# facebookresearch/nonrigid_nerf

Hardware: AMD Instinct MI355X
Metric: rendered rays/sec (64+128 samples/ray) (higher is better)
Workload: dtype bf16

## Files before the change

include/nrnerf.h:

```cpp
#ifndef NRNERF_H
#define NRNERF_H

#include <stddef.h>
#include <stdint.h>

#ifdef __cplusplus
extern "C" {
#endif

#define NRNERF_ABI_VERSION 10
#define NRNERF_MAX_SAMPLES 1024

typedef enum nrnerf_status {
    NRNERF_OK = 0,
    NRNERF_ERR_INVALID = -1,
    NRNERF_ERR_UNSUPPORTED = -2,
    NRNERF_ERR_HIP = -3,
    NRNERF_ERR_WORKSPACE = -4,
    NRNERF_ERR_NOMEM = -5,
    NRNERF_ERR_INTERNAL = -6
} nrnerf_status;

typedef enum nrnerf_precision {
    NRNERF_PREC_F32 = 0,
// ... 30 lines not shown
    int32_t rigidity_depth;
    int32_t rigidity_hidden;
    const nrnerf_linear* network;
    const nrnerf_linear* rigidity_network;
} nrnerf_bender_desc;

typedef struct nrnerf_model_desc {
    uint32_t struct_size;
    int32_t precision;
    int32_t multires;
    int32_t multires_views;
    int32_t device;
    const nrnerf_bender_desc* bender;
    const nrnerf_mlp_desc* coarse;
    const nrnerf_mlp_desc* fine;
    int32_t exact_viewdirs;
    uint32_t flags;
} nrnerf_model_desc;

typedef enum nrnerf_model_flags {
    NRNERF_MODEL_FORCE_GENERIC = 1u << 0,
    NRNERF_MODEL_NO_X16_F16 = 1u << 1
} nrnerf_model_flags;

typedef struct nrnerf_model nrnerf_model;

typedef struct nrnerf_sample_outputs {
    float* visibility_weights;
    float* opacity_alpha;
    float* initial_input_pts;
    float* unmasked_offsets;
    float* masked_offsets;
    float* input_pts;
    float* rigidity_mask;
} nrnerf_sample_outputs;

typedef struct nrnerf_render_args {
    uint32_t struct_size;
    int32_t n_rays;
    int32_t n_samples;
    int32_t n_importance;
    const float* rays;
    int32_t ray_stride;
    const float* latents;
    int32_t latent_stride;
    int32_t has_rigidity_cutoff;   float rigidity_cutoff;
    int32_t has_test_time_scaling; float test_time_scaling;
    int32_t has_removal_threshold; float removal_threshold;
    int32_t detailed_output;
    float* rgb_map;
    float* disp_map;
    float* acc_map;
    float* raw;
    float* rgb0;
    float* disp0;
    float* acc0;
    float* z_std;
    float* z_vals;
    float* surface_pts;
    float* surface_rigidity;
    int32_t* median_index;
    nrnerf_sample_outputs coarse;
    nrnerf_sample_outputs fine;
    void* workspace;
    size_t workspace_bytes;
    int32_t lindisp;
    int32_t white_bkgd;
    const float* u_coarse;
    const float* noise_coarse;
    const float* u_fine;
    const float* noise_fine;
    uint32_t flags;
} nrnerf_render_args;

typedef enum nrnerf_render_flags {
    NRNERF_RENDER_FUSED_FINE_BENDER = 1u << 0,
    NRNERF_RENDER_UNFUSED_COMPOSITE = 1u << 1,
    NRNERF_RENDER_SPLIT_COARSE = 1u << 2,
    NRNERF_RENDER_NO_X16 = 1u << 3,
    NRNERF_RENDER_X16_FINE_ONLY = 1u << 4,
    NRNERF_RENDER_BENDER_32X32 = 1u << 5,
    NRNERF_RENDER_COARSE_EPILOGUE_ON = 1u << 6,
    NRNERF_RENDER_COARSE_EPILOGUE_OFF = 1u << 7,
    NRNERF_RENDER_FIXED_SHARES = 1u << 8
} nrnerf_render_flags;

#define NRNERF_NUM_KERNELS 6
typedef struct nrnerf_profile {
    double ms[NRNERF_NUM_KERNELS];
    int64_t launches[NRNERF_NUM_KERNELS];
    double flops[NRNERF_NUM_KERNELS];
    double mfma_flops[NRNERF_NUM_KERNELS];
    char kernel_name[NRNERF_NUM_KERNELS][64];
} nrnerf_profile;

int nrnerf_abi_version(void);
const char* nrnerf_strerror(int status);

int nrnerf_model_create(const nrnerf_model_desc* desc, nrnerf_model** out);
int nrnerf_model_update(nrnerf_model* model, const nrnerf_model_desc* desc, void* hip_stream);
int64_t nrnerf_model_flat_size(const nrnerf_model* model);
int nrnerf_model_update_device(nrnerf_model* model, const float* flat_params, int64_t n_floats, void* hip_stream);
#define NRNERF_ADAM_MAX_SEGMENTS 40
typedef struct nrnerf_adam_segment {
    float* param; const float* grad; float* exp_avg; float* exp_avg_sq;
    uint64_t n;
} nrnerf_adam_segment;
typedef struct nrnerf_adam_args {
    uint32_t struct_size;
    int32_t n_segments;
    nrnerf_adam_segment segments[NRNERF_ADAM_MAX_SEGMENTS];
    float lr, beta1, beta2, eps;
    const float* lr_device;
    float* step;
    const float* flat_params;
    int64_t n_floats;
    uint32_t* barrier;
} nrnerf_adam_args;
int nrnerf_adam_step(nrnerf_model* model, const nrnerf_adam_args* args, void* hip_stream);

typedef struct nrnerf_tn_job {
    const void* a; const void* b;
    int32_t lda, ldb, wo, wi;
    int32_t ldo, reserved;
    int64_t out_offset, bias_offset;
} nrnerf_tn_job;
typedef struct nrnerf_tn_args {
    uint32_t struct_size;
    int32_t n_jobs, is_bf16, reserved;
    int64_t n_rows, out_floats;
    const nrnerf_tn_job* jobs;
    float* out;
    void* workspace; size_t workspace_bytes;
} nrnerf_tn_args;
size_t nrnerf_tn_workspace_bytes(const nrnerf_tn_args* args);
int nrnerf_tn_products(const nrnerf_tn_args* args, void* hip_stream);

typedef struct nrnerf_encoding_args {
    uint32_t struct_size;
    int32_t n_freqs;
    int64_t n_rows;
    const float* src; int32_t src_stride;
    void* enc; int32_t enc_cols; int32_t enc_is_bf16;
    const float* codes; int32_t n_lat; int32_t rows_per_code;
    const float* d_enc0; const float* d_enc1; int32_t d_enc_stride;
    float* d_src; int32_t d_src_stride;
} nrnerf_encoding_args;
int nrnerf_encoding_forward(const nrnerf_encoding_args* args, void* hip_stream);
int nrnerf_encoding_backward(const nrnerf_encoding_args* args, void* hip_stream);
void nrnerf_model_destroy(nrnerf_model* model);
int nrnerf_model_precision(const nrnerf_model* model);
int nrnerf_model_is_generic(const nrnerf_model* model);

size_t nrnerf_workspace_bytes(const nrnerf_model* model, int32_t n_rays, int32_t n_samples,
                              int32_t n_importance);

int nrnerf_render(const nrnerf_model* model, const nrnerf_render_args* args, void* hip_stream);

typedef struct nrnerf_camera {
    float c2w[12];
    float focal_x, focal_y, center_x, center_y;
    int32_t height, width;
} nrnerf_camera;
int nrnerf_generate_rays(const nrnerf_camera* cam, float near_plane, float far_plane, float* rays_out,
                         int32_t ray_stride, void* hip_stream);

int nrnerf_sample_depths(const float* rays, int32_t ray_stride, const float* uniforms, int32_t n_rays, int32_t n_samples,
// ... 123 lines not shown
    void* encv;
    float* head_sums;
} nrnerf_wgrad_args;
#define NRNERF_WGRAD_STRIDE_VIEWS(depth, width) (NRNERF_WGRAD_STRIDE(depth, width) + ((width) / 2) * (width) + 2 * ((width) / 2) * 64 + (width) / 2)
#define NRNERF_WGRAD_SHORT_PARTIALS(n_partials, width) \
    ((((n_partials) * (2 * ((width) / 64) + 2) + (2 * ((width) / 64) + (width) / 32) / 2) / (2 * ((width) / 64) + (width) / 32)) < 1 ? 1 : \
     (((n_partials) * (2 * ((width) / 64) + 2) + (2 * ((width) / 64) + (width) / 32) / 2) / (2 * ((width) / 64) + (width) / 32)))
#define NRNERF_WGRAD_STRIDE(depth, width) (((depth) - 1) * (width) * (width) + 3 * (width) * 64 + ((depth) + 1) * (width))
int nrnerf_trunk_wgrad(const nrnerf_model* model, const nrnerf_wgrad_args* args, void* hip_stream);

typedef struct nrnerf_generic_trunk_args {
    uint32_t struct_size;
    int32_t which;
    int32_t n_rays, n_samples;
    const float* pts4;
    void* acts;
    float* raw4;
    float* raw; int32_t raw_ch;
    const float* d_raw4;
    void* d_pre;
    float* d_enc0;
    float* d_enc1;
    const float* dirs;
    float* d_encv;
    const float* latents;
    void* relu_bits;
} nrnerf_generic_trunk_args;
size_t nrnerf_generic_trunk_bits_bytes(const nrnerf_model* model, int32_t which, int32_t n_rays, int32_t n_samples);
int nrnerf_generic_trunk_forward(const nrnerf_model* model, const nrnerf_generic_trunk_args* args, void* hip_stream);
int nrnerf_generic_trunk_backward(const nrnerf_model* model, const nrnerf_generic_trunk_args* args, void* hip_stream);
int nrnerf_model_trains_generic(const nrnerf_model* model);
int nrnerf_model_trains_bender(const nrnerf_model* model);

typedef struct nrnerf_loss_args {
    uint32_t struct_size;
    int32_t n_rays, n_samples;
    const float* rgb_map;
    const float* rgb0;
    const float* target;
    const float* weights;
    const float* offsets;
    const float* rigidity;
    const float* alpha;
    const float* divergence;
    float offsets_weight, rigidity_weight, divergence_weight;
    const float* schedule;
    float* loss;
    const float* g_loss;
    float* g_rgb_map;
    float* g_rgb0;
    float* g_offsets;
    float* g_rigidity;
    float* g_divergence;
    int32_t offsets_stride;
    int32_t rigidity_stride;
    const float* g_mean;
} nrnerf_loss_args;
int nrnerf_loss_forward(const nrnerf_loss_args* args, void* hip_stream);
int nrnerf_loss_backward(const nrnerf_loss_args* args, void* hip_stream);

int nrnerf_code_gradients(const int64_t* index, const float* g, int32_t n_rays, int32_t latent_size, int32_t n_codes, float* out, void* hip_stream);

typedef struct nrnerf_composite_args {
    uint32_t struct_size;
    int32_t n_rays, n_samples, n_importance;
    const float* rays; int32_t ray_stride;
    const float* raw4;
    const float* z;
    int32_t lindisp, white_bkgd;
    const float* noise;
    const float* u;
    float* rgb; float* disp; float* acc;
    float* weights; float* alpha;
    float* z_std; float* z_merged;
    const float* g_rgb; const float* g_disp; const float* g_acc; const float* g_weights;
    float* d_raw4;
    float* z_new;
    uint8_t* rank_new;
} nrnerf_composite_args;
int nrnerf_composite_forward(const nrnerf_composite_args* args, void* hip_stream);
int nrnerf_composite_backward(const nrnerf_composite_args* args, void* hip_stream);

int nrnerf_profile_begin(nrnerf_model* model);
int nrnerf_profile_end(nrnerf_model* model, nrnerf_profile* out);

typedef enum nrnerf_visualize_flags {
    NRNERF_VIS_DISP = 1, NRNERF_VIS_DISP_JET = 2, NRNERF_VIS_DISP_PHONG = 4,
    NRNERF_VIS_CORRESPONDENCES = 8, NRNERF_VIS_RIGIDITY = 16, NRNERF_VIS_RIGIDITY_JET = 32
} nrnerf_visualize_flags;
typedef enum nrnerf_visualize_normalize {
    NRNERF_VIS_NORM_NONE = 0,
    NRNERF_VIS_NORM_GIVEN = 1,
    NRNERF_VIS_NORM_FRAME = 2,
    NRNERF_VIS_NORM_STACK = 3
} nrnerf_visualize_normalize;
typedef struct nrnerf_visualize_args {
    uint32_t struct_size;
    uint32_t flags;
    int32_t n_frames, height, width;
    int32_t normalize;
    const float* disp;
    float* disp_max;
    const float* surface_pts;
    double min_point[3], max_point[3];
    int32_t voxels;
    const float* rigidity;
    uint8_t* disp_out;
    uint8_t* disp_jet;
    uint8_t* disp_phong;
    uint8_t* correspondences;
    uint8_t* rigidity_out;
    uint8_t* rigidity_jet;
} nrnerf_visualize_args;
int nrnerf_visualize_frames(const nrnerf_visualize_args* args, void* hip_stream);

typedef struct nrnerf_metrics_args {
    uint32_t struct_size;
    int32_t n_frames, height, width;
    const float* gt;
    const float* rendered;
    const float* mask_ref;
    double* psnr;
    double* ssim;
    double* mse;
    double* ssim_map;
    uint8_t* mse_error_map;
    uint8_t* ssim_error_map;
    void* workspace;
    size_t workspace_bytes;
} nrnerf_metrics_args;
size_t nrnerf_visualize_workspace_bytes(int32_t n_frames, int32_t height, int32_t width);
int nrnerf_image_metrics(const nrnerf_metrics_args* args, void* hip_stream);

int nrnerf_stability_accumulate(const float* rgb, int64_t n_values, double* sum, double* sum_sq, void* hip_stream);
int nrnerf_stability_finish(const double* sum, const double* sum_sq, int32_t n_frames, int64_t n_pixels, uint8_t* out_rgb, void* hip_stream);

typedef struct nrnerf_query_args {
    uint32_t struct_size;
    int32_t which;
    int32_t n_rows;
    int32_t n_samples;
    const float* points;
    int32_t point_stride;
    int32_t latent_stride;
    const float* latents;
    const float* viewdirs;
    int32_t has_rigidity_cutoff;   float rigidity_cutoff;
    int32_t has_test_time_scaling; float test_time_scaling;
    int32_t has_removal_threshold; float removal_threshold;
    int32_t detailed_output;
    uint32_t flags;
    int32_t raw_ch;
    float* raw;
    nrnerf_sample_outputs details;
    void* workspace;
    size_t workspace_bytes;
} nrnerf_query_args;
size_t nrnerf_query_workspace_bytes(const nrnerf_model* model, int32_t which, int32_t n_rows, int32_t n_samples);
int nrnerf_query(const nrnerf_model* model, const nrnerf_query_args* args, void* hip_stream);

int nrnerf_grid_points(const float min_point[3], const float max_point[3], int32_t gx, int32_t gy, int32_t gz, int64_t first_row,
                       int32_t n_rows, float* pts4, void* hip_stream);
int nrnerf_field_from_raw(const float* raw, int32_t raw_ch, int64_t n, float* sigma, uint8_t* rgb8, void* hip_stream);

typedef struct nrnerf_isosurface_args {
    uint32_t struct_size;
// ... 246 lines not shown
```

nonrigid_nerf_amd/_lib.py:

```python
from __future__ import annotations

import ctypes as C
import os

_HERE = os.path.dirname(os.path.abspath(__file__))
LIB_PATH = os.environ.get("NRNERF_LIB") or os.path.join(_HERE, "lib", "libnrnerf_hip.so")

ABI_VERSION = 10
MAX_SAMPLES = 1024
OK, ERR_INVALID, ERR_UNSUPPORTED, ERR_HIP, ERR_WORKSPACE, ERR_NOMEM, ERR_INTERNAL = 0, -1, -2, -3, -4, -5, -6
PRECISIONS = {"f32": 0, "fp32": 0, "float32": 0, "bf16": 1, "bfloat16": 1, "f16": 2, "fp16": 2, "float16": 2}
_CANONICAL = {0: "f32", 1: "bf16", 2: "f16"}


def canonical_precision(p: str) -> str:
    try:
        return _CANONICAL[PRECISIONS[p]]
    except KeyError:
        raise ValueError(f"unknown precision {p!r} (one of {sorted(PRECISIONS)})") from None
NUM_KERNELS = 6
KERNEL_NAMES = ("net_coarse", "composite_sample_coarse", "net_fine", "composite_fine", "bend_fine", "bend_coarse")

_fp = C.POINTER(C.c_float)


class Linear(C.Structure):
    _fields_ = [("weight", _fp), ("bias", _fp), ("out_features", C.c_int32), ("in_features", C.c_int32)]


class MlpDesc(C.Structure):
    _fields_ = [("depth", C.c_int32), ("width", C.c_int32), ("skip", C.c_int32), ("output_ch", C.c_int32),
                ("use_viewdirs", C.c_int32), ("time_conditioned", C.c_int32),
                ("pts_linears", C.POINTER(Linear)),
                ("output_linear", Linear), ("alpha_linear", Linear), ("feature_linear", Linear),
                ("views_linear", Linear), ("rgb_linear", Linear)]


class BenderDesc(C.Structure):
    _fields_ = [("latent_size", C.c_int32), ("depth", C.c_int32), ("hidden", C.c_int32),
                ("rigidity_depth", C.c_int32), ("rigidity_hidden", C.c_int32),
                ("network", C.POINTER(Linear)), ("rigidity_network", C.POINTER(Linear))]


class ModelDesc(C.Structure):
    _fields_ = [("struct_size", C.c_uint32), ("precision", C.c_int32), ("multires", C.c_int32),
                ("multires_views", C.c_int32), ("device", C.c_int32),
                ("bender", C.POINTER(BenderDesc)), ("coarse", C.POINTER(MlpDesc)), ("fine", C.POINTER(MlpDesc)),
                ("exact_viewdirs", C.c_int32), ("flags", C.c_uint32)]


class SampleOutputs(C.Structure):
    _fields_ = [(n, C.c_void_p) for n in ("visibility_weights", "opacity_alpha", "initial_input_pts",
                                           "unmasked_offsets", "masked_offsets", "input_pts", "rigidity_mask")]


class RenderArgs(C.Structure):
    _fields_ = [("struct_size", C.c_uint32), ("n_rays", C.c_int32), ("n_samples", C.c_int32),
                ("n_importance", C.c_int32),
                ("rays", C.c_void_p), ("ray_stride", C.c_int32),
                ("latents", C.c_void_p), ("latent_stride", C.c_int32),
                ("has_rigidity_cutoff", C.c_int32), ("rigidity_cutoff", C.c_float),
                ("has_test_time_scaling", C.c_int32), ("test_time_scaling", C.c_float),
                ("has_removal_threshold", C.c_int32), ("removal_threshold", C.c_float),
                ("detailed_output", C.c_int32),
                ("rgb_map", C.c_void_p), ("disp_map", C.c_void_p), ("acc_map", C.c_void_p), ("raw", C.c_void_p),
                ("rgb0", C.c_void_p), ("disp0", C.c_void_p), ("acc0", C.c_void_p), ("z_std", C.c_void_p),
                ("z_vals", C.c_void_p),
                ("surface_pts", C.c_void_p), ("surface_rigidity", C.c_void_p), ("median_index", C.c_void_p),
                ("coarse", SampleOutputs), ("fine", SampleOutputs),
                ("workspace", C.c_void_p), ("workspace_bytes", C.c_size_t),
                ("lindisp", C.c_int32), ("white_bkgd", C.c_int32),
                ("u_coarse", C.c_void_p), ("noise_coarse", C.c_void_p), ("u_fine", C.c_void_p), ("noise_fine", C.c_void_p),
                ("flags", C.c_uint32)]


MODEL_FORCE_GENERIC, MODEL_NO_X16_F16 = 1 << 0, 1 << 1
MODEL_PY_TRAINING_HANDLE = 1 << 30
RENDER_FUSED_FINE_BENDER, RENDER_UNFUSED_COMPOSITE, RENDER_SPLIT_COARSE, RENDER_NO_X16, RENDER_X16_FINE_ONLY, RENDER_BENDER_32X32, \
    RENDER_COARSE_EPILOGUE_ON, RENDER_COARSE_EPILOGUE_OFF, RENDER_FIXED_SHARES = (1 << i for i in range(9))


def model_flags_from_env() -> int:
    f = 0
    if os.environ.get("NRNERF_FORCE_GENERIC") == "1":
        f |= MODEL_FORCE_GENERIC
    if os.environ.get("NRNERF_X16_F16", "1") == "0":
        f |= MODEL_NO_X16_F16
    return f


_RENDER_ENV = ("NRNERF_FUSED_FINE_BENDER", "NRNERF_UNFUSED_COMPOSITE", "NRNERF_SPLIT_COARSE", "NRNERF_X16_BENDER", "NRNERF_X16",
               "NRNERF_FUSED_COARSE_EPILOGUE", "NRNERF_FIXED_SHARES")
_render_flags_cache = (None, 0)


def render_flags_from_env() -> int:
    global _render_flags_cache
    key = tuple(os.environ.get(k) for k in _RENDER_ENV)
    if _render_flags_cache[0] == key:
        return _render_flags_cache[1]
    f = 0
    if key[0] == "1":
        f |= RENDER_FUSED_FINE_BENDER
    if key[1] == "1":
        f |= RENDER_UNFUSED_COMPOSITE
    if key[2] == "1":
        f |= RENDER_SPLIT_COARSE
    if key[3] == "0":
        f |= RENDER_BENDER_32X32
    x16 = key[4]
    if x16 is not None and x16.strip() != "":
        if x16.strip() not in ("0", "1", "2"):
            raise ValueError(f"NRNERF_X16={x16!r}: one of 0 (32x32x16 kernels), 1 (16x16x32 fine pass only), 2 (both passes, the default)")
        f |= {0: RENDER_NO_X16, 1: RENDER_X16_FINE_ONLY}.get(int(x16), 0)
    if key[5] is not None and key[5].strip() != "":
        if key[5].strip() not in ("0", "1"):
            raise ValueError(f"NRNERF_FUSED_COARSE_EPILOGUE={key[5]!r}: 0 (composite / sample_pdf / merge as their own launch) or 1 (inside the coarse trunk kernel)")
        f |= RENDER_COARSE_EPILOGUE_ON if key[5].strip() == "1" else RENDER_COARSE_EPILOGUE_OFF
    if key[6] == "1":
        f |= RENDER_FIXED_SHARES
    _render_flags_cache = (key, f)
    return f


class GenericTrunkArgs(C.Structure):
    _fields_ = [("struct_size", C.c_uint32), ("which", C.c_int32), ("n_rays", C.c_int32), ("n_samples", C.c_int32),
                ("pts4", C.c_void_p), ("acts", C.c_void_p), ("raw4", C.c_void_p), ("raw", C.c_void_p), ("raw_ch", C.c_int32),
                ("d_raw4", C.c_void_p), ("d_pre", C.c_void_p), ("d_enc0", C.c_void_p), ("d_enc1", C.c_void_p),
                ("dirs", C.c_void_p), ("d_encv", C.c_void_p), ("latents", C.c_void_p), ("relu_bits", C.c_void_p)]


class LossArgs(C.Structure):
    _fields_ = [("struct_size", C.c_uint32), ("n_rays", C.c_int32), ("n_samples", C.c_int32),
                ("rgb_map", C.c_void_p), ("rgb0", C.c_void_p), ("target", C.c_void_p),
                ("weights", C.c_void_p), ("offsets", C.c_void_p), ("rigidity", C.c_void_p), ("alpha", C.c_void_p), ("divergence", C.c_void_p),
                ("offsets_weight", C.c_float), ("rigidity_weight", C.c_float), ("divergence_weight", C.c_float), ("schedule", C.c_void_p),
                ("loss", C.c_void_p), ("g_loss", C.c_void_p),
                ("g_rgb_map", C.c_void_p), ("g_rgb0", C.c_void_p), ("g_offsets", C.c_void_p), ("g_rigidity", C.c_void_p), ("g_divergence", C.c_void_p),
                ("offsets_stride", C.c_int32), ("rigidity_stride", C.c_int32), ("g_mean", C.c_void_p)]


class Profile(C.Structure):
    _fields_ = [("ms", C.c_double * NUM_KERNELS), ("launches", C.c_int64 * NUM_KERNELS),
                ("flops", C.c_double * NUM_KERNELS), ("mfma_flops", C.c_double * NUM_KERNELS),
                ("kernel_name", (C.c_char * 64) * NUM_KERNELS)]


class PackedInfo(C.Structure):
    _fields_ = [("stream_bytes", C.c_uint64), ("n_units", C.c_uint32), ("n_bias_tiles", C.c_uint32),
                ("frag_bytes", C.c_uint32), ("slot_bytes", C.c_uint32), ("mfma_per_block", C.c_uint32)]


class Camera(C.Structure):
    _fields_ = [("c2w", C.c_float * 12), ("focal_x", C.c_float), ("focal_y", C.c_float), ("center_x", C.c_float),
                ("center_y", C.c_float), ("height", C.c_int32), ("width", C.c_int32)]


class TrunkArgs(C.Structure):
    _fields_ = [("struct_size", C.c_uint32), ("which", C.c_int32), ("n_rays", C.c_int32), ("n_samples", C.c_int32),
                ("pts4", C.c_void_p), ("acts", C.c_void_p), ("relu_mask", C.c_void_p),
                ("raw4", C.c_void_p), ("raw", C.c_void_p), ("raw_ch", C.c_int32),
                ("d_raw4", C.c_void_p), ("d_pre", C.c_void_p), ("d_pts4", C.c_void_p), ("ray_bias", C.c_void_p),
                ("dirs", C.c_void_p), ("hv", C.c_void_p), ("hv_mask", C.c_void_p), ("d_pre_v", C.c_void_p), ("d_dirs", C.c_void_p)]


class WgradArgs(C.Structure):
    _fields_ = [("struct_size", C.c_uint32), ("n_rays", C.c_int32), ("n_samples", C.c_int32),
                ("acts", C.c_void_p), ("d_pre", C.c_void_p), ("pts4", C.c_void_p), ("d_raw4", C.c_void_p),
                ("enc", C.c_void_p), ("g_head", C.c_void_p),
                ("n_partials", C.c_int32), ("partials", C.c_void_p),
                ("dirs", C.c_void_p), ("hv", C.c_void_p), ("d_pre_v", C.c_void_p), ("encv", C.c_void_p), ("head_sums", C.c_void_p)]


REDUCE_SHORT = 0x40000000


def wgrad_stride(depth: int, width: int) -> int:
    return (depth - 1) * width * width + 3 * width * 64 + (depth + 1) * width


def wgrad_stride_views(depth: int, width: int) -> int:
    return wgrad_stride(depth, width) + (width // 2) * width + 2 * (width // 2) * 64 + width // 2


def wgrad_short_partials(n_partials: int, width: int) -> int:
    trw = width // 64
    return min(n_partials, max(1, (n_partials * (2 * trw + 2) + (2 * trw + width // 32) // 2) // (2 * trw + width // 32)))


class BenderArgs(C.Structure):
    _fields_ = [("struct_size", C.c_uint32), ("n_rays", C.c_int32), ("n_samples", C.c_int32),
                ("rays", C.c_void_p), ("ray_stride", C.c_int32),
                ("latents", C.c_void_p), ("latent_stride", C.c_int32),
                ("z", C.c_void_p),
                ("has_rigidity_cutoff", C.c_int32), ("rigidity_cutoff", C.c_float),
                ("has_test_time_scaling", C.c_int32), ("test_time_scaling", C.c_float),
                ("bent4", C.c_void_p), ("off4", C.c_void_p), ("acts_offsets", C.c_void_p), ("acts_rigidity", C.c_void_p),
                ("g_bent4", C.c_void_p), ("g_unmasked_offsets", C.c_void_p), ("g_rigidity_mask", C.c_void_p),
                ("dz_offsets", C.c_void_p), ("dz_rigidity", C.c_void_p), ("dz_out4", C.c_void_p), ("d_latents", C.c_void_p),
                ("g_bent4_b", C.c_void_p)]


class BenderWgradArgs(C.Structure):
# ... 203 lines not shown
                ("flags", C.c_uint32), ("bent4", C.c_void_p),
                ("workspace", C.c_void_p), ("workspace_bytes", C.c_size_t)]


BEND_POINTS_WORKSPACE_BYTES = 512 * 64


ISO_BLOCK, ISO_SCAN_CHUNK, ISO_MAX_VERTICES = 256, 4096, 1 << 30


def isosurface_workspace_bytes(gx: int, gy: int, gz: int) -> int:
    n = gx * gy * gz
    if min(gx, gy, gz) < 2 or n > ISO_MAX_VERTICES:
        return 0
    nb = (n + ISO_BLOCK - 1) // ISO_BLOCK
    return sum((b + 255) // 256 * 256 for b in (4 * n, 4 * nb, 4 * nb, 8 * nb, 8 * nb, n))


EXPORTS = {
    "nrnerf_abi_version": (C.c_int, []),
    "nrnerf_strerror": (C.c_char_p, [C.c_int]),
    "nrnerf_model_create": (C.c_int, [C.POINTER(ModelDesc), C.POINTER(C.c_void_p)]),
    "nrnerf_model_update": (C.c_int, [C.c_void_p, C.c_void_p, C.c_void_p]),
    "nrnerf_model_flat_size": (C.c_int64, [C.c_void_p]),
    "nrnerf_model_update_device": (C.c_int, [C.c_void_p, C.c_void_p, C.c_int64, C.c_void_p]),
    "nrnerf_adam_step": (C.c_int, [C.c_void_p, C.POINTER(AdamArgs), C.c_void_p]),
    "nrnerf_tn_workspace_bytes": (C.c_size_t, [C.POINTER(TnArgs)]),
    "nrnerf_tn_products": (C.c_int, [C.POINTER(TnArgs), C.c_void_p]),
    "nrnerf_encoding_forward": (C.c_int, [C.POINTER(EncodingArgs), C.c_void_p]),
    "nrnerf_encoding_backward": (C.c_int, [C.POINTER(EncodingArgs), C.c_void_p]),
    "nrnerf_model_destroy": (None, [C.c_void_p]),
    "nrnerf_model_precision": (C.c_int, [C.c_void_p]),
    "nrnerf_model_is_generic": (C.c_int, [C.c_void_p]),
    "nrnerf_generic_trunk_forward": (C.c_int, [C.c_void_p, C.POINTER(GenericTrunkArgs), C.c_void_p]),
    "nrnerf_generic_trunk_backward": (C.c_int, [C.c_void_p, C.POINTER(GenericTrunkArgs), C.c_void_p]),
    "nrnerf_model_trains_generic": (C.c_int, [C.c_void_p]),
    "nrnerf_generic_trunk_bits_bytes": (C.c_size_t, [C.c_void_p, C.c_int32, C.c_int32, C.c_int32]),
    "nrnerf_model_trains_bender": (C.c_int, [C.c_void_p]),
    "nrnerf_loss_forward": (C.c_int, [C.POINTER(LossArgs), C.c_void_p]),
    "nrnerf_loss_backward": (C.c_int, [C.POINTER(LossArgs), C.c_void_p]),
    "nrnerf_code_gradients": (C.c_int, [C.c_void_p, C.c_void_p, C.c_int32, C.c_int32, C.c_int32, C.c_void_p, C.c_void_p]),
    "nrnerf_workspace_bytes": (C.c_size_t, [C.c_void_p, C.c_int32, C.c_int32, C.c_int32]),
    "nrnerf_render": (C.c_int, [C.c_void_p, C.POINTER(RenderArgs), C.c_void_p]),
    "nrnerf_query_workspace_bytes": (C.c_size_t, [C.c_void_p, C.c_int32, C.c_int32, C.c_int32]),
    "nrnerf_query": (C.c_int, [C.c_void_p, C.POINTER(QueryArgs), C.c_void_p]),
    "nrnerf_grid_points": (C.c_int, [_fp, _fp, C.c_int32, C.c_int32, C.c_int32, C.c_int64, C.c_int32, C.c_void_p, C.c_void_p]),
    "nrnerf_field_from_raw": (C.c_int, [C.c_void_p, C.c_int32, C.c_int64, C.c_void_p, C.c_void_p, C.c_void_p]),
    "nrnerf_isosurface_workspace_bytes": (C.c_size_t, [C.c_int32, C.c_int32, C.c_int32]),
    "nrnerf_isosurface_count": (C.c_int, [C.POINTER(IsosurfaceArgs), C.c_void_p]),
    "nrnerf_isosurface_emit": (C.c_int, [C.POINTER(IsosurfaceArgs), C.c_void_p]),
    "nrnerf_bender_inverse_workspace_bytes": (C.c_size_t, [C.c_void_p]),
    "nrnerf_bender_inverse": (C.c_int, [C.c_void_p, C.POINTER(BenderInverseArgs), C.c_void_p]),
    "nrnerf_volume_render": (C.c_int, [C.POINTER(VolumeRenderArgs), C.c_void_p]),
    "nrnerf_warped_volume_render": (C.c_int, [C.POINTER(WarpedVolumeRenderArgs), C.c_void_p]),
    "nrnerf_grid_lookup_backward": (C.c_int, [C.POINTER(GridLookupBackwardArgs), C.c_void_p]),
    "nrnerf_sh_volume_render": (C.c_int, [C.POINTER(ShVolumeRenderArgs), C.c_void_p]),
    "nrnerf_occupancy_words": (C.c_int64, [C.POINTER(C.c_int32), C.c_int32]),
    "nrnerf_occupancy_build": (C.c_int, [C.POINTER(OccupancyBuildArgs), C.c_void_p]),
    "nrnerf_culled_volume_render": (C.c_int, [C.POINTER(CulledVolumeRenderArgs), C.c_void_p]),
    "nrnerf_bend_points_workspace_bytes": (C.c_size_t, [C.c_void_p]),
    "nrnerf_bend_points": (C.c_int, [C.c_void_p, C.POINTER(BendPointsArgs), C.c_void_p]),
    "nrnerf_generate_rays": (C.c_int, [C.POINTER(Camera), C.c_float, C.c_float, C.c_void_p, C.c_int32, C.c_void_p]),
    "nrnerf_sample_depths": (C.c_int, [C.c_void_p, C.c_int32, C.c_void_p, C.c_int32, C.c_int32, C.c_int32, C.c_void_p, C.c_void_p]),
    "nrnerf_sample_depths_points": (C.c_int, [C.c_void_p, C.c_int32, C.c_void_p, C.c_int32, C.c_int32, C.c_int32, C.c_void_p, C.c_void_p, C.c_void_p]),
    "nrnerf_merge_rows": (C.c_int, [C.c_void_p, C.c_int32, C.c_int32, C.c_int32, C.c_void_p, C.c_void_p, C.c_void_p, C.c_void_p, C.c_void_p, C.c_void_p,
                                    C.c_int32, C.c_void_p]),
    "nrnerf_reduce_partials": (C.c_int, [C.c_void_p, C.c_int64, C.c_int32, C.c_int32, C.c_void_p, C.c_int64, C.c_void_p, C.c_void_p]),
    "nrnerf_reduce_partials_aux": (C.c_int, [C.c_void_p, C.c_int64, C.c_int32, C.c_int32, C.c_void_p, C.c_int64, C.c_void_p, C.c_void_p, C.c_int32,
                                             C.POINTER(C.c_int64), C.c_void_p]),
    "nrnerf_tile_row_sums": (C.c_int, [C.c_void_p, C.c_int64, C.c_void_p, C.c_void_p]),
    "nrnerf_tiles_to_rows": (C.c_int, [C.c_void_p, C.c_int32, C.c_int32, C.c_int32, C.c_void_p, C.c_void_p]),
    "nrnerf_direction_encoding": (C.c_int, [C.c_void_p, C.c_int32, C.c_int32, C.c_int32, C.c_void_p, C.c_int32, C.c_void_p, C.c_void_p]),
    "nrnerf_trunk_forward": (C.c_int, [C.c_void_p, C.POINTER(TrunkArgs), C.c_void_p]),
    "nrnerf_trunk_backward": (C.c_int, [C.c_void_p, C.POINTER(TrunkArgs), C.c_void_p]),
    "nrnerf_trunk_wgrad": (C.c_int, [C.c_void_p, C.POINTER(WgradArgs), C.c_void_p]),
    "nrnerf_bender_forward": (C.c_int, [C.c_void_p, C.POINTER(BenderArgs), C.c_void_p]),
    "nrnerf_bender_backward": (C.c_int, [C.c_void_p, C.POINTER(BenderArgs), C.c_void_p]),
    "nrnerf_bender_wgrad": (C.c_int, [C.c_void_p, C.POINTER(BenderWgradArgs), C.c_void_p]),
    "nrnerf_bender_divergence_forward": (C.c_int, [C.c_void_p, C.POINTER(DivergenceArgs), C.c_void_p]),
    "nrnerf_bender_divergence_backward": (C.c_int, [C.c_void_p, C.POINTER(DivergenceArgs), C.c_void_p]),
    "nrnerf_composite_forward": (C.c_int, [C.POINTER(CompositeArgs), C.c_void_p]),
    "nrnerf_composite_backward": (C.c_int, [C.POINTER(CompositeArgs), C.c_void_p]),
    "nrnerf_profile_begin": (C.c_int, [C.c_void_p]),
    "nrnerf_profile_end": (C.c_int, [C.c_void_p, C.POINTER(Profile)]),
    "nrnerf_visualize_frames": (C.c_int, [C.POINTER(VisualizeArgs), C.c_void_p]),
    "nrnerf_visualize_workspace_bytes": (C.c_size_t, [C.c_int32, C.c_int32, C.c_int32]),
    "nrnerf_image_metrics": (C.c_int, [C.POINTER(MetricsArgs), C.c_void_p]),
    "nrnerf_stability_accumulate": (C.c_int, [C.c_void_p, C.c_int64, C.c_void_p, C.c_void_p, C.c_void_p]),
    "nrnerf_stability_finish": (C.c_int, [C.c_void_p, C.c_void_p, C.c_int32, C.c_int64, C.c_void_p, C.c_void_p]),
    "nrnerf_pack_host": (C.c_int, [C.POINTER(ModelDesc), C.c_int, C.POINTER(PackedInfo), C.c_void_p, C.c_size_t,
                                   C.POINTER(C.c_uint32), _fp]),
}

_lib = None


class NrnerfError(RuntimeError):
    def __init__(self, status: int, where: str):
        self.status = status
        super().__init__(f"{where}: {strerror(status)} (status {status})")


def load() -> C.CDLL:
    global _lib
    if _lib is None:
        if not os.path.exists(LIB_PATH):
            raise ImportError(
                f"{LIB_PATH} not found: build it with `python -c 'import __graft_entry__ as g; g.build()'` "
                "(or `make -C nonrigid_nerf_amd/csrc -j8`). nonrigid_nerf_amd has no CPU fallback.")
        import torch
        lib = C.CDLL(LIB_PATH)
        for name, (res, args) in EXPORTS.items():
            fn = getattr(lib, name)
            fn.restype, fn.argtypes = res, args
        v = lib.nrnerf_abi_version()
        if v != ABI_VERSION:
            raise ImportError(f"libnrnerf_hip.so ABI version {v}, binding expects {ABI_VERSION}")
        _lib = lib
    return _lib


def strerror(status: int) -> str:
    return load().nrnerf_strerror(status).decode()


def check(status: int, where: str):
    if status != OK:
        raise NrnerfError(status, where)
```

nonrigid_nerf_amd/csrc/nrnerf_api.cpp:

```cpp
#include <hip/hip_runtime.h>

#include <cstdio>
#include <cstring>
#include <mutex>
#include <new>
#include <vector>

#include "nrnerf_model.h"
#include "nrnerf_aux.h"
#include "nrnerf_x16_api.h"
#include "nrnerf_plan.h"
#include "nrnerf_bend_points.h"
#include "nrnerf_field.h"

using namespace nrn;

namespace {

int upload_pass(const PackedPass& pk, PassDev& dev) {
    dev.stream_bytes = pk.stream.size();
    dev.bias_floats = pk.bias.size();
    if (hipMalloc(&dev.stream, pk.stream.size()) != hipSuccess) return NRNERF_ERR_NOMEM;
    if (hipMalloc((void**)&dev.bias, pk.bias.size() * 4) != hipSuccess) return NRNERF_ERR_NOMEM;
    if (hipMemcpy(dev.stream, pk.stream.data(), pk.stream.size(), hipMemcpyHostToDevice) != hipSuccess) return NRNERF_ERR_HIP;
// ... 344 lines not shown
    }
    template <class F> hipError_t timed(nrnerf_model::Ev ev, F&& launch) {
        if (!prof) return launch();
        if (hipEventCreateWithFlags(&ev.a, hipEventDisableSystemFence) != hipSuccess ||
            hipEventCreateWithFlags(&ev.b, hipEventDisableSystemFence) != hipSuccess) return hipErrorUnknown;
        (void)hipEventRecord(ev.a, stream);
        const hipError_t e = launch();
        (void)hipEventRecord(ev.b, stream);
        std::lock_guard<std::mutex> g(m->prof_mu);
        m->prof_events.push_back(ev);
        return e;
    }
    hipError_t run_program(const nrnerf_model::Ev& ev, const GenArgs& g) { return timed(ev, [&] { return launch_generic(m->precision, g, m->num_cus, stream); }); }
    static SampleOut sample_out(const nrnerf_sample_outputs& o) {
        return SampleOut{o.visibility_weights, o.opacity_alpha, o.initial_input_pts, o.unmasked_offsets, o.masked_offsets, o.input_pts, o.rigidity_mask};
    }
    const nrnerf_sample_outputs& outputs_of(const PassPlan& p) const { return p.which ? a->fine : a->coarse; }
    const float* depths_of(const PassPlan& p) const { return p.which ? z_fine : zc; }
    float* points_of(const PassPlan& p) const { return p.final ? bent4_ws : bent_c; }
    float* raw_of(const PassPlan& p) const { return p.which ? raw_f : raw_c; }

    hipError_t bender_step(const PassPlan& p) {
        const float* const zv = p.bend_rank ? z_new : depths_of(p);
        if (p.bend == BendStep::Program) {
            const ImageDev& im = m->gen_bend;
            GenArgs g = im.prog;
            g.rays = a->rays; g.ray_stride = a->ray_stride; g.latents = a->latents; g.lat_stride = a->latent_stride;
            g.z = zv; g.lindisp = a->lindisp; g.n_rays = N; g.S = p.bend_n;
            g.wstream = im.stream; g.bias = im.bias;
            g.bent4 = points_of(p); g.ex = sample_out(outputs_of(p)); g.knobs = kn;
            return run_program(work(p.bend_slot, "gen_kernel (bender program)", im, p.bend_n), g);
        }
        const ImageDev& im = plan.bend_x16 ? m->bend_x16 : m->bend_only;
        BendArgs b{};
        b.rays = a->rays; b.ray_stride = a->ray_stride; b.latents = a->latents; b.lat_stride = a->latent_stride;
        b.z = zv; b.lindisp = a->lindisp; b.rank = p.bend_rank ? rank_new : nullptr; b.n_rays = N; b.n_per_ray = p.bend_n; b.out_stride = p.bend_stride;
        b.wstream = im.stream; b.bias = im.bias; b.bent4 = points_of(p); b.knobs = kn;
        b.work_counter = counter(p.bend_dynamic, (size_t)16 * BEND_COUNTERS_PER_LAUNCH * p.which);
        return timed(work(p.bend_slot, plan.bend_x16 ? "bend_kernel_x16" : "bend_kernel", im, p.bend_n), [&] {
            return plan.bend_x16 ? launch_bend_x16(bender_arch_of(m), b, m->num_cus, stream) : launch_bend(m->precision, bender_arch_of(m), b, m->num_cus, stream);
        });
    }
    CompositeArgs composite_args(const PassPlan& p) const {
        const bool fine = p.which == 1;
        const nrnerf_sample_outputs& so = outputs_of(p);
        CompositeArgs c{};
        c.rays = a->rays; c.ray_stride = a->ray_stride;
        c.raw4 = raw_of(p); c.z = depths_of(p); c.n_rays = N; c.S = p.S; c.n_importance = p.final ? 0 : I;
        c.lindisp = a->lindisp; c.white_bkgd = a->white_bkgd; c.noise = fine ? a->noise_fine : a->noise_coarse;
        c.vis = so.visibility_weights; c.alpha = so.opacity_alpha;
        if (p.final) {
            c.rgb = a->rgb_map; c.disp = a->disp_map; c.acc = a->acc_map; c.z_user = a->z_vals;
            if (plan.surface) { c.bent4 = bent4_ws; c.surf_pts = a->surface_pts; c.surf_rig = a->surface_rigidity; c.med_idx = a->median_index; }
        } else {
            c.u = a->u_fine;
            c.rgb = a->rgb0 ? a->rgb0 : raw_f; c.disp = a->disp0 ? a->disp0 : raw_f + (size_t)N * 3; c.acc = a->acc0 ? a->acc0 : raw_f + (size_t)N * 4;
            c.z_std = a->z_std; c.z_out = z_fine;
            if (plan.split) { c.split_bent_in = bent_c; c.split_bent_out = bent4_ws; c.z_new = z_new; c.rank_new = rank_new; }
        }
        return c;
    }
    hipError_t network_step(const PassPlan& p, const CompositeArgs& c) {
        const bool fused = p.comp != CompStep::Launch;
        const ImageDev& im = m->img[p.image];
        const nrnerf_sample_outputs& so = outputs_of(p);
        const float* const pts = given_pts ? given_pts : ((p.bend == BendStep::Compiled || p.bend == BendStep::Program) ? points_of(p) : nullptr);
        float* const pts_out = (!pts && (p.final ? plan.surface : plan.split)) ? points_of(p) : nullptr;
        float* const raw4 = fused ? nullptr : raw_of(p);
        float* const raw_out = p.final ? a->raw : nullptr;
        CompositeArgs fuse = fused ? c : CompositeArgs{};
        fuse.raw4 = nullptr;
        const nrnerf_model::Ev ev = work(p.net_slot, p.name, im, p.S);
        switch (p.net) {
        case NetFamily::NetBender: case NetFamily::NetTrunk: case NetFamily::NetX16: {
            NetArgs n{};
            n.rays = a->rays; n.ray_stride = a->ray_stride; n.latents = a->latents; n.lat_stride = a->latent_stride;
            n.z = depths_of(p); n.lindisp = a->lindisp; n.pts4 = pts; n.n_rays = N; n.S = p.S;
            n.wstream = im.stream; n.bias = im.bias;
            n.raw4 = raw4; n.raw_out = raw_out; n.raw_ch = im.output_ch; n.bent4 = pts_out;
            n.ex = sample_out(so); n.knobs = kn; n.fuse_on = fused; n.fuse = fuse;
            return timed(ev, [&] {
                if (p.net != NetFamily::NetX16) return launch_net(m->precision, p.net == NetFamily::NetBender, m->views, p.dispatch, n, m->num_cus, stream);
                n.work_counter = counter(p.trunk_counter, (size_t)16 * BEND_COUNTERS_PER_LAUNCH * 2 + 16 * p.which);
                return launch_net_x16(m->precision, p.dispatch, m->views, n, m->num_cus, stream);
            });
        }
        case NetFamily::Gx16: {
            const GxMeta& gm = im.gx;
            GxArgs x{};
            x.pts4 = pts; x.raw4 = raw4; x.raw_out = raw_out; x.raw_ch = im.output_ch;
            x.n_rays = N; x.S = p.S; x.wstream = im.stream; x.bias = im.bias;
            x.depth = gm.depth; x.skip = gm.skip; x.L = gm.L; x.n_bias_tiles = gm.n_bias_tiles; x.LV = gm.LV;
            x.fuse_on = fused; x.fuse = fuse;
            return timed(ev, [&] { return launch_gx16(m->precision, p.dispatch, gm.views != 0, x, m->num_cus, stream); });
        }
        case NetFamily::Gen: {
            GenArgs g = im.prog;
            g.rays = a->rays; g.ray_stride = a->ray_stride; g.latents = a->latents; g.lat_stride = a->latent_stride;
            g.z = depths_of(p); g.lindisp = a->lindisp; g.n_rays = N; g.S = p.S;
            g.pts4 = pts; g.dirs_from_pts = (pts && m->views && m->has_bend) ? 1 : 0;
            g.wstream = im.stream; g.bias = im.bias;
            g.raw4 = raw4; g.raw_out = raw_out; g.raw_ch = im.output_ch;
            g.bent4 = pts ? const_cast<float*>(pts) : pts_out;
            g.knobs = kn;
            if (!pts) g.ex = sample_out(so);
            return run_program(ev, g);
        }
        case NetFamily::GenExact: {
            BendDivArgs t{};
            t.latents = a->latents; t.lat_stride = a->latent_stride; t.m = (long long)N * p.S;
            t.wstream = m->bend_train_fwd.stream; t.bias = m->bend_train_fwd.bias;
            t.knobs.has_cutoff = kn.has_cutoff; t.knobs.cutoff = kn.cutoff; t.knobs.has_scaling = kn.has_scaling; t.knobs.scaling = kn.scaling;
            t.rays = a->rays; t.ray_stride = a->ray_stride; t.zr = depths_of(p); t.S = p.S; t.lindisp = a->lindisp; t.dirs_out = jdirs;
            const bool b16 = m->precision != NRNERF_PREC_F32;
            const hipError_t je = (m->gen_compiled_bender == 0) ? launch_bend_div_fwd_a0(t, m->num_cus, stream, b16) : launch_bend_div_fwd_a1(t, m->num_cus, stream, b16);
            if (je != hipSuccess) return je;
            GenArgs g = im.prog;
            g.mode = 1;
            g.rays = pts; g.ray_stride = 0; g.latents = nullptr; g.lat_stride = 0;
            g.z = nullptr; g.lindisp = 0; g.n_rays = N; g.S = p.S;
            g.pts4 = pts; g.dirs_from_pts = 0; g.dirs = jdirs;
            g.wstream = im.stream; g.bias = im.bias;
            g.raw4 = raw4; g.raw_out = raw_out; g.raw_ch = im.output_ch; g.bent4 = const_cast<float*>(pts);
            g.save = nullptr; g.mask = nullptr; g.save_stride = 0; g.save_w = 0;
            g.knobs = kn;
            return timed(ev, [&] { return launch_generic_train(m->precision, g, m->num_cus, stream); });
        }
        }
        return hipErrorUnknown;
    }
    int run_pass(const PassPlan& p) {
        if ((p.bend == BendStep::Compiled || p.bend == BendStep::Program) && bender_step(p) != hipSuccess) return NRNERF_ERR_HIP;
        const CompositeArgs c = composite_args(p);
        if (network_step(p, c) != hipSuccess) return NRNERF_ERR_HIP;
        if (p.comp != CompStep::Launch) return NRNERF_OK;
        const nrnerf_model::Ev ev{p.net_slot + 1, nullptr, nullptr, 0, 0, "composite_kernel"};
        return status_of(timed(ev, [&] { return launch_composite(c, stream); }));
    }
};
}
extern "C" {

int nrnerf_render(const nrnerf_model* m, const nrnerf_render_args* a, void* hip_stream) try {
    if (!m || !a || a->struct_size != sizeof(nrnerf_render_args)) return NRNERF_ERR_INVALID;
    if (a->n_rays < 0 || a->n_samples < 2 || a->n_importance < 0) return NRNERF_ERR_INVALID;
    if (a->n_samples > NRNERF_MAX_SAMPLES || a->n_samples + a->n_importance > NRNERF_MAX_SAMPLES) return NRNERF_ERR_UNSUPPORTED;
    if (a->n_rays == 0) return NRNERF_OK;
    if (!a->rays || a->ray_stride < 8 || !a->rgb_map || !a->disp_map || !a->acc_map) return NRNERF_ERR_INVALID;
    if (m->needs_latents && (!a->latents || a->latent_stride < 0)) return NRNERF_ERR_INVALID;
    if (m->views && (!m->has_bend || m->exact) && a->ray_stride < 11) return NRNERF_ERR_INVALID;
    const size_t need = nrnerf_workspace_bytes(m, a->n_rays, a->n_samples, a->n_importance);
    if (!a->workspace || a->workspace_bytes < need || ((uintptr_t)a->workspace & 255)) return NRNERF_ERR_WORKSPACE;
    hipStream_t stream = (hipStream_t)hip_stream;
    DeviceGuard guard(m->device);
    if (!guard.ok) return NRNERF_ERR_HIP;
    const WorkspaceLayout lay(a->n_rays, a->n_samples, a->n_importance, m->generic && m->exact);
    if ((a->u_fine || a->noise_fine) && a->n_importance == 0) return NRNERF_ERR_INVALID;
    const RenderPlan plan = plan_render(*m, *a);
    RenderCall call(m, a, plan, lay, stream);
    if (plan.counters_first) (void)call.counter(true, 0);
    if (a->u_coarse) {
        JitterArgs ja{a->rays, a->ray_stride, a->u_coarse, a->n_rays, a->n_samples, a->lindisp, call.z_coarse};
        if (launch_zjitter(ja, stream) != hipSuccess) return NRNERF_ERR_HIP;
        call.zc = call.z_coarse;
    }
    const int rc = call.run_pass(plan.coarse);
// ... 129 lines not shown
        r.n_rays = (int32_t)M; r.n_samples = 1; r.rays = pk.point_records;
        if (q.point_latents) { r.latents = pk.latents_out; r.latent_stride = m->latent_size; }
    }
    RenderPlan rp;
    rp.generic = m->generic != 0; rp.bend_x16 = q.bend_x16;
    RenderCall call(m, &r, rp, stream, raw4, pts4, (unsigned*)(ws + lay.counters));
    if (p.bend_dynamic) (void)call.counter(true, 0);
    if (!q.per_point && !m->has_bend) call.given_pts = pts4;

    if (p.bend == BendStep::Compiled) {
        const ImageDev& bi = q.bend_x16 ? m->bend_x16 : m->bend_only;
        BendPointArgs b{};
        b.b.latents = a->latents; b.b.lat_stride = a->latent_stride; b.b.n_rays = N; b.b.n_per_ray = S; b.b.out_stride = S;
        b.b.wstream = bi.stream; b.b.bias = bi.bias; b.b.bent4 = pts4; b.b.knobs = call.kn;
        b.b.work_counter = call.counter(p.bend_dynamic, (size_t)16 * BEND_COUNTERS_PER_LAUNCH * p.which);
        b.src.points = a->points; b.src.stride = a->point_stride; b.src.unmasked = d.unmasked_offsets; b.src.masked = d.masked_offsets;
        const hipError_t e = call.timed(call.work(p.bend_slot, q.bend_x16 ? "bend_kernel_x16 (point source)" : "bend_kernel (point source)", bi, S), [&] {
            return q.bend_x16 ? launch_bend_points_x16(bender_arch_of(m), b, m->num_cus, stream)
                              : launch_bend_points(m->precision, bender_arch_of(m), b, m->num_cus, stream);
        });
        if (e != hipSuccess) return NRNERF_ERR_HIP;
    }
    if (call.network_step(p, CompositeArgs{}) != hipSuccess) return NRNERF_ERR_HIP;
    if (m->has_bend) {
        QueryUnpackArgs u{};
        u.bent4 = pts4; u.n = M; u.in_pts = d.input_pts; u.rigidity = d.rigidity_mask;
        u.raw = a->raw; u.raw_ch = a->raw_ch; u.has_removal = a->detailed_output && a->has_removal_threshold; u.removal = a->removal_threshold;
        if ((u.in_pts || u.rigidity || u.has_removal) && launch_query_unpack(u, stream) != hipSuccess) return NRNERF_ERR_HIP;
    }
    return NRNERF_OK;
} NRN_CATCH

int nrnerf_grid_points(const float min_point[3], const float max_point[3], int32_t gx, int32_t gy, int32_t gz, int64_t first_row,
                       int32_t n_rows, float* pts4, void* hip_stream) try {
    if (!min_point || !max_point || gx < 1 || gy < 1 || gz < 1 || first_row < 0 || n_rows < 0) return NRNERF_ERR_INVALID;
    if (first_row + n_rows > (int64_t)gy * gz) return NRNERF_ERR_INVALID;
    if (n_rows == 0) return NRNERF_OK;
    if (!pts4) return NRNERF_ERR_INVALID;
    GridArgs g{};
    for (int c = 0; c < 3; ++c) { g.lo[c] = min_point[c]; g.hi[c] = max_point[c]; }
    g.g[0] = gx; g.g[1] = gy; g.g[2] = gz; g.first_row = first_row; g.n_rows = n_rows; g.pts4 = pts4;
    return on_owner_of(pts4, [&] { return status_of(launch_grid_points(g, (hipStream_t)hip_stream)); });
} NRN_CATCH

int nrnerf_field_from_raw(const float* raw, int32_t raw_ch, int64_t n, float* sigma, uint8_t* rgb8, void* hip_stream) try {
    if (n < 0 || raw_ch < 4) return NRNERF_ERR_INVALID;
    if (n == 0 || (!sigma && !rgb8)) return NRNERF_OK;
    if (!raw) return NRNERF_ERR_INVALID;
    return on_owner_of(raw, [&] { return status_of(launch_field_from_raw(raw, raw_ch, n, sigma, rgb8, (hipStream_t)hip_stream)); });
} NRN_CATCH

int nrnerf_generate_rays(const nrnerf_camera* cam, float near_plane, float far_plane, float* rays_out,
                         int32_t ray_stride, void* hip_stream) try {
    if (!cam || !rays_out || (ray_stride != 8 && ray_stride != 11)) return NRNERF_ERR_INVALID;
    if (cam->height <= 0 || cam->width <= 0 || cam->focal_x == 0.0f || cam->focal_y == 0.0f) return NRNERF_ERR_INVALID;
    RayGenArgs a{};
    std::memcpy(a.c2w, cam->c2w, sizeof(a.c2w));
    a.fx = cam->focal_x; a.fy = cam->focal_y; a.cx = cam->center_x; a.cy = cam->center_y;
    a.H = cam->height; a.W = cam->width; a.near = near_plane; a.far = far_plane;
    a.rays = rays_out; a.ray_stride = ray_stride;
    return on_owner_of(rays_out, [&] { return status_of(launch_raygen(a, (hipStream_t)hip_stream)); });
} NRN_CATCH

int nrnerf_sample_depths(const float* rays, int32_t ray_stride, const float* uniforms, int32_t n_rays, int32_t n_samples,
                         int32_t lindisp, float* z_out, void* hip_stream) try {
    if (!rays || !z_out || ray_stride < 8 || n_rays < 0 || n_samples < 2 || n_samples > NRNERF_MAX_SAMPLES) return NRNERF_ERR_INVALID;
    if (n_rays == 0) return NRNERF_OK;
    const JitterArgs j{rays, ray_stride, uniforms, n_rays, n_samples, lindisp, z_out};
    return on_owner_of(z_out, [&] { return status_of(launch_zjitter(j, (hipStream_t)hip_stream)); });
} NRN_CATCH
int nrnerf_sample_depths_points(const float* rays, int32_t ray_stride, const float* uniforms, int32_t n_rays, int32_t n_samples,
                                int32_t lindisp, float* z_out, float* points_out, void* hip_stream) try {
    if (!rays || !z_out || !points_out || ray_stride < 8 || n_rays < 0 || n_samples < 2 || n_samples > NRNERF_MAX_SAMPLES) return NRNERF_ERR_INVALID;
    if (n_rays == 0) return NRNERF_OK;
    const SamplePointsArgs j{rays, ray_stride, uniforms, n_rays, n_samples, lindisp, z_out, points_out};
    return on_owner_of(z_out, [&] { return status_of(launch_sample_points(j, (hipStream_t)hip_stream)); });
} NRN_CATCH

int nrnerf_profile_begin(nrnerf_model* m) try {
    if (!m) return NRNERF_ERR_INVALID;
    std::lock_guard<std::mutex> g(m->prof_mu);
    for (auto& e : m->prof_events) { (void)hipEventDestroy(e.a); (void)hipEventDestroy(e.b); }
    m->prof_events.clear();
    m->prof_on = true;
    return NRNERF_OK;
} NRN_CATCH

int nrnerf_profile_end(nrnerf_model* m, nrnerf_profile* out) try {
    if (!m || !out) return NRNERF_ERR_INVALID;
    std::lock_guard<std::mutex> g(m->prof_mu);
    m->prof_on = false;
    std::memset(out, 0, sizeof(*out));
    int rc = NRNERF_OK;
    for (auto& e : m->prof_events) {
        float ms = 0.f;
        if (hipEventSynchronize(e.b) != hipSuccess || hipEventElapsedTime(&ms, e.a, e.b) != hipSuccess) rc = NRNERF_ERR_HIP;
        out->ms[e.kernel] += ms;
        out->launches[e.kernel] += 1;
        out->flops[e.kernel] += e.flops;
        out->mfma_flops[e.kernel] += e.mfma;
        if (e.name) std::snprintf(out->kernel_name[e.kernel], sizeof(out->kernel_name[e.kernel]), "%s", e.name);
        (void)hipEventDestroy(e.a); (void)hipEventDestroy(e.b);
    }
    m->prof_events.clear();
    return rc;
} NRN_CATCH

}
```

nonrigid_nerf_amd/csrc/nrnerf_kernels.h:

```cpp
#pragma once
#include <hip/hip_runtime.h>
#include <stdint.h>

#include <type_traits>

namespace nrn {

constexpr int epl_class(int S) {
    const int n = (S + 63) / 64;
    return n <= 4 ? n : n <= 6 ? 6 : n <= 8 ? 8 : n <= 12 ? 12 : 16;
}
static_assert(epl_class(1) == 1 && epl_class(64) == 1 && epl_class(65) == 2 && epl_class(128) == 2 && epl_class(129) == 3 && epl_class(192) == 3 &&
              epl_class(193) == 4 && epl_class(256) == 4 && epl_class(257) == 6 && epl_class(384) == 6 && epl_class(385) == 8 && epl_class(512) == 8 &&
              epl_class(513) == 12 && epl_class(768) == 12 && epl_class(769) == 16 && epl_class(1024) == 16, "the lane-width table");
template <class F>
auto with_epl(int S, F&& f) {
    switch (epl_class(S)) {
        case 1: return f(std::integral_constant<int, 1>{});
        case 2: return f(std::integral_constant<int, 2>{});
        case 3: return f(std::integral_constant<int, 3>{});
        case 4: return f(std::integral_constant<int, 4>{});
        case 6: return f(std::integral_constant<int, 6>{});
        case 8: return f(std::integral_constant<int, 8>{});
        case 12: return f(std::integral_constant<int, 12>{});
        default: return f(std::integral_constant<int, 16>{});
    }
}

struct SampleOut {
    float* vis;
    float* alpha;
    float* init_pts;
    float* unmasked;
    float* masked;
    float* in_pts;
    float* rigidity;
};

struct Knobs {
    int has_cutoff;  float cutoff;
    int has_scaling; float scaling;
    int has_removal; float removal;
    int detailed;
};

struct CompositeArgs {
    const float* rays;   int ray_stride;
    const float* raw4;
    const float* z;
    int lindisp;
    int white_bkgd;
    const float* noise;
    const float* u;
    int n_rays, S;
    int n_importance;
    float* rgb; float* disp; float* acc;
    float* z_std;
    float* z_out;
    float* z_user;
    float* vis; float* alpha;
    const float* bent4;
    float* surf_pts;
    float* surf_rig;
    int* med_idx;
    const float* split_bent_in;
    float* split_bent_out;
    float* z_new;
    uint8_t* rank_new;
};

struct NetArgs {
    const float* rays;   int ray_stride;
    const float* latents; int lat_stride;
    const float* z;
    int lindisp;
    const float* pts4;
    int n_rays, S;
    const void* wstream;
    const float* bias;
    float* raw4;
    float* raw_out;
    int raw_ch;
    float* bent4;
    SampleOut ex;
    Knobs knobs;
    int fuse_on;
    CompositeArgs fuse;
    unsigned* work_counter;
};



struct BendArgs {
    const float* rays;   int ray_stride;
    const float* latents; int lat_stride;
    const float* z;
    int lindisp;
    const uint8_t* rank;
    int n_rays, n_per_ray, out_stride;
    const void* wstream;
    const float* bias;
    float* bent4;
    Knobs knobs;
    unsigned* work_counter;
};
hipError_t launch_bend(int precision, int arch_id, const BendArgs& a, int num_cus, hipStream_t stream);

struct CompositeBwdArgs {
    const float* rays;   int ray_stride;
    const float* raw4;
    const float* z;
    int lindisp, white_bkgd;
    const float* noise;
    int n_rays, S;
    const float* g_rgb;
    const float* g_disp;
    const float* g_acc;
    const float* g_w;
    float* d_raw4;
};
hipError_t launch_composite_bwd(const CompositeBwdArgs& a, hipStream_t stream);

struct TrunkArgs {
    const float* pts4;
    int n_rays, S;
    const void* wstream;
    const float* bias;
    float* raw4;
    float* raw_out;
    int raw_ch;
    void* acts;
    unsigned short* mask;
    const float* d_raw4;
    const float* ray_bias;
    void* d_pre;
    float* d_pts4;
    const float* dirs;
    void* hv;
    unsigned short* hv_mask;
    void* d_pre_v;
    float* d_dirs;
};

hipError_t launch_trunk_fwd_train_f32(const TrunkArgs&, int num_cus, hipStream_t);
hipError_t launch_trunk_fwd_train_bf16(const TrunkArgs&, int num_cus, hipStream_t);
hipError_t launch_trunk_bwd_f32(const TrunkArgs&, int num_cus, hipStream_t);
hipError_t launch_trunk_bwd_bf16(const TrunkArgs&, int num_cus, hipStream_t);
hipError_t launch_trunk_fwd_train_f32_views(const TrunkArgs&, int num_cus, hipStream_t);
hipError_t launch_trunk_fwd_train_bf16_views(const TrunkArgs&, int num_cus, hipStream_t);
hipError_t launch_trunk_bwd_f32_views(const TrunkArgs&, int num_cus, hipStream_t);
hipError_t launch_trunk_bwd_bf16_views(const TrunkArgs&, int num_cus, hipStream_t);
hipError_t launch_trunk_fwd_train_f32_a5(const TrunkArgs&, int num_cus, hipStream_t);
hipError_t launch_trunk_fwd_train_bf16_a5(const TrunkArgs&, int num_cus, hipStream_t);
hipError_t launch_trunk_bwd_f32_a5(const TrunkArgs&, int num_cus, hipStream_t);
hipError_t launch_trunk_bwd_bf16_a5(const TrunkArgs&, int num_cus, hipStream_t);

struct BendTrainArgs {
    const float* rays;   int ray_stride;
    const float* latents; int lat_stride;
    const float* z;
    int n_rays, S;
    const void* wstream;
    const float* bias;
    Knobs knobs;
    float* bent4;
    float* off4;
    void* acts_b;
    void* acts_r;
    const float* g_bent4;
    const float* g_bent4_b;
    const float* g_unmasked;
// ... 192 lines not shown
```

nonrigid_nerf_amd/csrc/nrnerf_model.h:

```cpp
#pragma once
#include <hip/hip_runtime.h>

#include <mutex>
#include <new>
#include <vector>

#include "nrnerf_pack.h"

#define NRN_CATCH catch (const std::bad_alloc&) { return NRNERF_ERR_NOMEM; } catch (...) { return NRNERF_ERR_INTERNAL; }

struct PassDev {
    void* stream = nullptr;
    float* bias = nullptr;
    size_t stream_bytes = 0, bias_floats = 0;
    double algo_flops_per_sample = 0;
    double mfma_flops_per_sample = 0;
    int output_ch = 4;
    int32_t* src = nullptr; int32_t* bias_src = nullptr; uint8_t* fmt = nullptr;
    size_t n_elems = 0;
};

struct ImageDev : PassDev { nrn::GenArgs prog{}; nrn::GxMeta gx{}; };

struct DeviceGuard {
    int prev = -1;
    bool ok = true;
    explicit DeviceGuard(int want) {
        if (hipGetDevice(&prev) != hipSuccess) { ok = false; prev = -1; return; }
        if (prev != want && hipSetDevice(want) != hipSuccess) ok = false;
        if (prev == want) prev = -1;
    }
    ~DeviceGuard() { if (prev >= 0) (void)hipSetDevice(prev); }
};

struct nrnerf_model : nrn::ModelTraits {
    explicit nrnerf_model(const nrn::ModelTraits& t)
        : nrn::ModelTraits(t), fine(img[t.fine_is_coarse ? nrn::IMG_COARSE : nrn::IMG_FINE]), gen_fine(img[t.fine_is_coarse ? nrn::IMG_GEN_COARSE : nrn::IMG_GEN_FINE]) {}
    int device = 0, num_cus = 0;
    ImageDev img[nrn::IMG_COUNT];
    ImageDev &coarse = img[nrn::IMG_COARSE], &fine;
    ImageDev &fine_trunk = img[nrn::IMG_FINE_TRUNK], &coarse_trunk = img[nrn::IMG_COARSE_TRUNK], &bend_only = img[nrn::IMG_BEND_ONLY];
    ImageDev &fine_trunk_x16 = img[nrn::IMG_FINE_TRUNK_X16], &coarse_trunk_x16 = img[nrn::IMG_COARSE_TRUNK_X16];
    ImageDev &bend_x16 = img[nrn::IMG_BEND_X16];
    ImageDev &coarse_bwd = img[nrn::IMG_COARSE_BWD], &fine_bwd = img[nrn::IMG_FINE_BWD];
    ImageDev &coarse_train = img[nrn::IMG_COARSE_TRAIN], &fine_train = img[nrn::IMG_FINE_TRAIN];
    ImageDev &bend_train_fwd = img[nrn::IMG_BEND_TRAIN_FWD], &bend_train_bwd = img[nrn::IMG_BEND_TRAIN_BWD];
    ImageDev &gen_bend = img[nrn::IMG_GEN_BEND], &gen_coarse = img[nrn::IMG_GEN_COARSE], &gen_fine;
    ImageDev &gx_coarse = img[nrn::IMG_GX_COARSE], &gx_fine = img[nrn::IMG_GX_FINE];
    ImageDev &gen_coarse_bwd = img[nrn::IMG_GEN_COARSE_BWD], &gen_fine_bwd = img[nrn::IMG_GEN_FINE_BWD];
    ImageDev &gx_coarse_bwd = img[nrn::IMG_GX_COARSE_BWD], &gx_fine_bwd = img[nrn::IMG_GX_FINE_BWD];
    int64_t flat_floats = 0;
    unsigned* adam_barrier = nullptr;
    mutable std::mutex prof_mu;
    mutable bool prof_on = false;
    struct Ev { int kernel; hipEvent_t a, b; double flops, mfma; const char* name; };
    mutable std::vector<Ev> prof_events;
};

namespace nrn { hipError_t launch_generic_train(int precision, const GenArgs& a, int num_cus, hipStream_t stream); }

inline int bender_arch_of(const nrnerf_model* m) { return m->generic ? m->gen_compiled_bender : nrn::bender_arch(m->arch_id); }

inline int device_of(const void* ptr, int& dev) {
    hipPointerAttribute_t attr;
    if (hipPointerGetAttributes(&attr, ptr) != hipSuccess) { (void)hipGetLastError(); return NRNERF_ERR_INVALID; }
    if (attr.type != hipMemoryTypeDevice) return NRNERF_ERR_INVALID;
    dev = attr.device;
    return NRNERF_OK;
}

inline int status_of(hipError_t e) { return e == hipSuccess ? NRNERF_OK : NRNERF_ERR_HIP; }
inline int status_of_checked_launch(hipError_t e) { return e == hipErrorInvalidValue ? NRNERF_ERR_INVALID : status_of(e); }

template <class RUN> int on_device(int dev, RUN&& run) {
    DeviceGuard guard(dev);
    if (!guard.ok) return NRNERF_ERR_HIP;
    return run();
}
template <class RUN> int on_owner_of(const void* ptr, RUN&& run) {
    int dev = 0;
    if (device_of(ptr, dev) != NRNERF_OK) return NRNERF_ERR_INVALID;
    return on_device(dev, run);
}
template <class RUN> int on_model_device(const nrnerf_model* m, RUN&& run) { return on_device(m->device, run); }

inline int repack_batches(const nrnerf_model* m, const float* flat_params, hipStream_t stream) {
    for (const ImageDev& p : m->img)
        if (p.stream && !p.src) return NRNERF_ERR_UNSUPPORTED;
    nrn::RepackBatchArgs b{};
    b.flat = flat_params;
    auto add = [&](const int32_t* src, const uint8_t* fmt, void* dst, long long n) -> bool {
        if (n <= 0) return true;
        if (b.n_segments == nrn::REPACK_MAX_SEGMENTS) {
            if (nrn::launch_repack_batch(b, stream) != hipSuccess) return false;
            b.n_segments = 0;
        }
        const int k = b.n_segments++;
        if (k == 0) b.block0[0] = 0;
        b.src[k] = src; b.fmt[k] = fmt; b.dst[k] = dst; b.n[k] = n;
        b.block0[k + 1] = b.block0[k] + (unsigned)((n + 255) / 256);
        return true;
    };
    for (const ImageDev& p : m->img) {
        if (!p.stream) continue;
        if (!add(p.src, p.fmt, p.stream, (long long)p.n_elems) || !add(p.bias_src, nullptr, p.bias, (long long)p.bias_floats)) return NRNERF_ERR_HIP;
    }
    return status_of(nrn::launch_repack_batch(b, stream));
}
```

nonrigid_nerf_amd/csrc/nrnerf_net_impl.h:

```cpp
#pragma once
#include <hip/hip_runtime.h>
#include <type_traits>

#include "nrnerf_kernels.h"
#include "nrnerf_plan.h"
#include "nrnerf_composite_ray.h"

#ifndef NRN_PF16
#define NRN_PF16 4
#endif
#ifndef NRN_EPI_DELAY
#define NRN_EPI_DELAY 4
#endif

namespace nrn {

#ifdef NRN_TIMING
static __device__ unsigned long long g_nrn_timing[8][8];
#define NRN_NOW() __builtin_amdgcn_s_memtime()
#define NRN_TACC(slot, t0) tacc[slot] += NRN_NOW() - (t0)
#else
#define NRN_NOW() 0ull
#define NRN_TACC(slot, t0) ((void)0)
#endif
// ... 2 lines not shown
typedef float f32x4 __attribute__((ext_vector_type(4)));

template <int I, int N, class F>
__device__ __forceinline__ void static_for(F&& f) {
    if constexpr (N - I == 1) {
        f(std::integral_constant<int, I>{});
    } else if constexpr (N - I > 1) {
        constexpr int M = I + (N - I) / 2;
        static_for<I, M>(f);
        static_for<M, N>(f);
    }
}

typedef short s16x8 __attribute__((ext_vector_type(8)));
typedef short s16x2 __attribute__((ext_vector_type(2)));
typedef float f32x2 __attribute__((ext_vector_type(2)));
typedef unsigned u32x4 __attribute__((ext_vector_type(4)));

template <class F8, class F2, int U, bool RELU>
__device__ __forceinline__ F8 pack16(const f32x16& c) {
    u32x4 w;
#pragma unroll
    for (int k = 0; k < 4; ++k) {
        const f32x2 t = {c[8 * U + 2 * k], c[8 * U + 2 * k + 1]};
        const F2 p = __builtin_convertvector(t, F2);
        s16x2 q = __builtin_bit_cast(s16x2, p);
        if (RELU) q = __builtin_elementwise_max(q, (s16x2)(short)0);
        w[k] = __builtin_bit_cast(unsigned, q);
    }
    return __builtin_bit_cast(F8, w);
}

__device__ __forceinline__ float relu_bits(float x) {
    return __builtin_bit_cast(float, max(__builtin_bit_cast(int, x), 0));
}
struct PolBF16 : Shape<8, false> {
    typedef __bf16 frag __attribute__((ext_vector_type(8)));
    static constexpr int PF = NRN_PF16;
    typedef __bf16 frag2 __attribute__((ext_vector_type(2)));
    template <int U, bool RELU>
    static __device__ __forceinline__ frag from_acc(const f32x16& c) { return pack16<frag, frag2, U, RELU>(c); }
    static __device__ __forceinline__ f32x16 mfma(frag a, frag b, f32x16 c) {
        return __builtin_amdgcn_mfma_f32_32x32x16_bf16(a, b, c, 0, 0, 0);
    }
    template <int E>
    static __device__ __forceinline__ void set(frag& f, float v) { f[E] = (__bf16)v; }
    static __device__ __forceinline__ float round(float v) { return (float)(__bf16)v; }
};
struct PolF16 : Shape<8, true> {
    typedef _Float16 frag __attribute__((ext_vector_type(8)));
    static constexpr int PF = NRN_PF16;
    typedef _Float16 frag2 __attribute__((ext_vector_type(2)));
    template <int U, bool RELU>
    static __device__ __forceinline__ frag from_acc(const f32x16& c) { return pack16<frag, frag2, U, RELU>(c); }
    static __device__ __forceinline__ f32x16 mfma(frag a, frag b, f32x16 c) {
        return __builtin_amdgcn_mfma_f32_32x32x16_f16(a, b, c, 0, 0, 0);
    }
    template <int E>
    static __device__ __forceinline__ void set(frag& f, float v) { f[E] = (_Float16)v; }
    static __device__ __forceinline__ float round(float v) { return (float)(_Float16)v; }
};
struct PolF32 : Shape<1> {
    typedef float frag;
    static constexpr int PF = 8;
    template <int U, bool RELU>
    static __device__ __forceinline__ frag from_acc(const f32x16& c) { return RELU ? relu_bits(c[U]) : c[U]; }
    static __device__ __forceinline__ f32x16 mfma(frag a, frag b, f32x16 c) {
        return __builtin_amdgcn_mfma_f32_32x32x2f32(a, b, c, 0, 0, 0);
    }
    template <int E>
    static __device__ __forceinline__ void set(frag& f, float v) { f = v; }
    static __device__ __forceinline__ float round(float v) { return v; }
};

#ifndef NRN_RING_LAG
#define NRN_RING_LAG 2
#endif
template <int N>
__device__ __forceinline__ void wait_ring() {
    if constexpr (NRN_RING_LAG == 1) asm volatile("s_waitcnt vmcnt(%0) lgkmcnt(0)" ::"n"(N) : "memory");
    else asm volatile("s_waitcnt vmcnt(%0)" ::"n"(N) : "memory");
}

template <class P, int WAVES, int NUP>
struct WRing {
    static constexpr int UNIT = P::UNIT_BYTES;
    static constexpr int PW = UNIT / 1024 / WAVES;
    static constexpr int LAG = NRN_RING_LAG;
    static_assert(LAG >= 1 && RING - LAG >= 2, "need at least one unit of DMA lead");
    static_assert(UNIT % (1024 * WAVES) == 0, "unit must split evenly over the waves");
    static_assert(NUP % RING == 0 && NUP >= RING, "unit count must be a padded multiple of the ring depth");
    const char* ubase;
    unsigned lane16;
    char* ring;
    int wave_off;
    int lane_off;
    unsigned lane_addr;
#ifdef NRN_TIMING
    unsigned long long bar_cycles = 0, bar_count = 0;
#endif

    __device__ __forceinline__ void init(const void* stream, char* lds, int wave, int lane) {
        wave_off = wave * PW * 1024;
        ubase = (const char*)stream + wave_off;
        lane16 = (unsigned)lane * 16u;
        ring = lds;
        lane_off = lane * (P::FRAG_BYTES / 64);
        lane_addr = (unsigned)(size_t)(__attribute__((address_space(3))) char*)lds + (unsigned)lane_off;
        static_for<0, RING - LAG>([&](auto uc) { issue<decltype(uc)::value>(); });
    }
    template <int V>
    __device__ __forceinline__ void issue() {
        unsigned off = (unsigned)(V * UNIT);
        asm volatile("" : "+s"(off));
        const char* src = (ubase + off) + lane16;
        char* dst = ring + (V % RING) * UNIT + wave_off;
        static_for<0, PW>([&](auto ic) {
            __builtin_amdgcn_global_load_lds((const __attribute__((address_space(1))) void*)src,
                                             (__attribute__((address_space(3))) void*)dst, 16, decltype(ic)::value * 1024, 0);
        });
    }
    template <int U>
    __device__ __forceinline__ void advance() {
#ifdef NRN_TIMING
        const unsigned long long tb0 = NRN_NOW();
#endif
        wait_ring<(RING - LAG - 1) * PW>();
        __builtin_amdgcn_s_barrier();
        asm volatile("" ::: "memory");
#ifdef NRN_TIMING
        bar_cycles += NRN_NOW() - tb0; ++bar_count;
#endif
        issue<(U + RING - LAG) % NUP>();
    }
    static constexpr bool ASM_FRAGS = (P::FRAG_BYTES == 1024);
    template <class PX, int GF>
    __device__ __forceinline__ typename PX::frag frag() {
        static_assert(PX::FRAG_BYTES == P::FRAG_BYTES, "mixed policies must share the fragment size");
        constexpr int UF = P::UNIT_FRAGS;
        if constexpr (GF % UF == 0) advance<GF / UF>();
        constexpr int OFF = ((GF / UF) % RING) * UNIT + (GF % UF) * P::FRAG_BYTES;
        if constexpr (ASM_FRAGS) {
            static_assert(OFF + 16 <= 65536, "ring must stay within the immediate ds_read offset");
            u32x4 v;
            asm volatile("ds_read_b128 %0, %1 offset:%2" : "=v"(v) : "v"(lane_addr), "n"(OFF));
            return __builtin_bit_cast(typename PX::frag, v);
        } else {
            const char* p = ring + OFF + lane_off;
            return *(const typename PX::frag*)p;
        }
    }
    template <int N, class F>
    __device__ __forceinline__ void ready(F& f) {
        if constexpr (ASM_FRAGS) {
            static_assert(N >= 0 && N <= 15, "lgkmcnt is a 4-bit counter");
            u32x4 v = __builtin_bit_cast(u32x4, f);
            asm volatile("s_waitcnt lgkmcnt(%1)" : "+v"(v) : "n"(N));
            f = __builtin_bit_cast(F, v);
        }
    }
    __device__ __forceinline__ void drain() { asm volatile("s_waitcnt vmcnt(0)" ::: "memory"); }
};

typedef const __attribute__((address_space(3))) f32x4* BiasPtr;
__device__ __forceinline__ BiasPtr bias_lane_ptr(const float* bias_lds, int h) {
    BiasPtr p = (BiasPtr)(bias_lds + h * 16);
    asm volatile("" : "+v"(p));
    return p;
}
__device__ __forceinline__ f32x16 load_bias(BiasPtr bias_lane, int tile) {
    BiasPtr bp = bias_lane + tile * 8;
    const f32x4 b0 = bp[0], b1 = bp[1], b2 = bp[2], b3 = bp[3];
    return f32x16{b0[0], b0[1], b0[2], b0[3], b1[0], b1[1], b1[2], b1[3],
                  b2[0], b2[1], b2[2], b2[3], b3[0], b3[1], b3[2], b3[3]};
}

template <int NT, int NS>
struct SeqPos {
    static constexpr int NPAIR = NT / 2;
    static constexpr int tile(int q) { return q < NPAIR * 2 * NS ? 2 * (q / (2 * NS)) + (q & 1) : NT - 1; }
    static constexpr int slab(int q) { return q < NPAIR * 2 * NS ? (q % (2 * NS)) / 2 : q - NPAIR * 2 * NS; }
    static constexpr bool last_of_tile(int q) { return slab(q) == NS - 1; }
};

#ifndef NRN_PRIO_HALF
#define NRN_PRIO_HALF 0
#endif
template <int Q>
__device__ __forceinline__ void prio_tick() {
    if constexpr (NRN_PRIO_HALF > 0) {
        if constexpr (Q % (2 * NRN_PRIO_HALF) == 0) __builtin_amdgcn_s_setprio(1);
        else if constexpr (Q % (2 * NRN_PRIO_HALF) == NRN_PRIO_HALF) __builtin_amdgcn_s_setprio(0);
    }
}

#ifndef NRN_NACC
#define NRN_NACC 2
#endif

template <class P0, class P1, class PL, int LI, int NS0, int NS1, class ST, class IN0, class IN1, class EPI>
__device__ __forceinline__ void dense(ST& st, BiasPtr bias_lane, const IN0& in0, const IN1& in1, EPI&& epi) {
    constexpr LayerSpec spec = PL::TB.layers[LI];
    static_assert(spec.ns == NS0 + NS1 && spec.split == 0, "slab count mismatch between kernel and plan");
    constexpr int NS = NS0 + NS1, NT = spec.nt, Q = NT * NS, PF = P1::PF;
    using SQ = SeqPos<NT, NS>;
    constexpr int G0 = PL::TB.tiles[spec.tile0].gbase;
    constexpr int NACC = (NT >= 4) ? NRN_NACC : (NT >= 2 ? 2 : 1);
    typename P1::frag a[PF];
    auto load = [&](auto qc) {
        constexpr int q = decltype(qc)::value;
        constexpr int s = SQ::slab(q);
        if constexpr (s < NS0) a[q % PF] = __builtin_bit_cast(typename P1::frag, st.template frag<P0, G0 + q>());
        else a[q % PF] = st.template frag<P1, G0 + q>();
    };
    static_for<0, (PF < Q ? PF : Q)>([&](auto qc) { load(qc); });
    constexpr int DLY = (NS - 1 < NRN_EPI_DELAY) ? NS - 1 : NRN_EPI_DELAY;
    f32x16 accs[NACC];
    static_for<0, (NACC < NT ? NACC : NT)>([&](auto tc) {
        constexpr int t = decltype(tc)::value;
        if constexpr (NACC == 4 || t < 2) accs[t % NACC] = load_bias(bias_lane, spec.tile0 + t);
    });
    static_for<0, Q>([&](auto qc) {
        constexpr int q = decltype(qc)::value;
        constexpr int t = SQ::tile(q), s = SQ::slab(q);
        prio_tick<q>();
        st.template ready<(Q - 1 - q < PF - 1) ? Q - 1 - q : PF - 1>(a[q % PF]);
        const typename P1::frag cur = a[q % PF];
        if constexpr (q + PF < Q) load(std::integral_constant<int, q + PF>{});
        if constexpr (s < NS0) accs[t % NACC] = P0::mfma(__builtin_bit_cast(typename P0::frag, cur), in0[s], accs[t % NACC]);
        else accs[t % NACC] = P1::mfma(cur, in1[s - NS0], accs[t % NACC]);
        if constexpr (NACC == 4) {
            if constexpr (t >= 2 && (t & 1) == 1 && s == DLY) {
                constexpr int tp = (t & ~1) - 2;
                epi(std::integral_constant<int, tp>{}, accs[tp % NACC]);
                epi(std::integral_constant<int, tp + 1>{}, accs[(tp + 1) % NACC]);
                if constexpr (tp + 4 < NT) accs[(tp + 4) % NACC] = load_bias(bias_lane, spec.tile0 + tp + 4);
                if constexpr (tp + 5 < NT) accs[(tp + 5) % NACC] = load_bias(bias_lane, spec.tile0 + tp + 5);
            }
            if constexpr (q == Q - 1) {
                constexpr int first = (NT & 1) ? (NT >= 3 ? NT - 3 : NT - 1) : NT - 2;
                static_for<first, NT>([&](auto tc) { epi(tc, accs[decltype(tc)::value % NACC]); });
            }
        } else {
            if constexpr (SQ::last_of_tile(q) && (((t & 1) == 1) || t == NT - 1)) {
// ... 715 lines not shown
```

nonrigid_nerf_amd/csrc/nrnerf_net_x16.h:

```cpp
#pragma once
#include "nrnerf_net_impl.h"
#include "nrnerf_composite_ray.h"

namespace nrn {

template <class P> struct X16;
template <> struct X16<PolBF16> {
    static __device__ __forceinline__ f32x4 mfma(PolBF16::frag a, PolBF16::frag b, f32x4 c) { return __builtin_amdgcn_mfma_f32_16x16x32_bf16(a, b, c, 0, 0, 0); }
};
template <> struct X16<PolF16> {
    static __device__ __forceinline__ f32x4 mfma(PolF16::frag a, PolF16::frag b, f32x4 c) { return __builtin_amdgcn_mfma_f32_16x16x32_f16(a, b, c, 0, 0, 0); }
};

template <class P>
__device__ __forceinline__ typename P::frag x16_pack(const f32x4& d0, const f32x4& d1) {
    typedef typename P::frag2 F2;
    u32x4 w;
#pragma unroll
    for (int k = 0; k < 4; ++k) {
        const f32x2 t = (k < 2) ? f32x2{d0[2 * k], d0[2 * k + 1]} : f32x2{d1[2 * (k - 2)], d1[2 * (k - 2) + 1]};
        s16x2 q = __builtin_bit_cast(s16x2, __builtin_convertvector(t, F2));
        q = __builtin_elementwise_max(q, (s16x2)(short)0);
        w[k] = __builtin_bit_cast(unsigned, q);
    }
    return __builtin_bit_cast(typename P::frag, w);
}

#ifndef NRN_X16_NB
#define NRN_X16_NB 4
#endif
#ifndef NRN_X16_WAVES
#define NRN_X16_WAVES 4
#endif
#ifndef NRN_X16_NB_NARROW
#define NRN_X16_NB_NARROW 4
#endif
#ifndef NRN_X16_WAVES_NARROW
#define NRN_X16_WAVES_NARROW 8
#endif
#ifndef NRN_X16_PF_NARROW
#define NRN_X16_PF_NARROW 2
#endif
#ifndef NRN_X16_PF
#define NRN_X16_PF 8
#endif

template <class A> struct X16Cfg {
    static constexpr int NB = (A::W <= 128) ? NRN_X16_NB_NARROW : NRN_X16_NB, WAVES = (A::W <= 128) ? NRN_X16_WAVES_NARROW : NRN_X16_WAVES;
    static constexpr int PF = (A::W <= 128) ? NRN_X16_PF_NARROW : NRN_X16_PF;
};
template <class P0, class P1, class PL, int LI, int NS0, int NS1, int NB, int PF_ = NRN_X16_PF, class ST, class IN0, class IN1, class EPI>
__device__ __forceinline__ void dense_x16(ST& st, const __attribute__((address_space(3))) f32x4* bias_lane, const IN0 (&in0)[NB], const IN1 (&in1)[NB],
                                          EPI&& epi) {
    constexpr LayerSpec spec = PL::TB.layers[LI];
    static_assert(spec.ns == NS0 + NS1, "k-step count mismatch between kernel and plan");
    constexpr int NS = NS0 + NS1, NT = spec.nt, Q = NT * NS, PF = PF_;
    using SQ = SeqPos<NT, NS>;
    constexpr int G0 = PL::TB.tiles[spec.tile0].gbase;
    typename P1::frag a[PF];
    f32x4 bias[NT];
    const unsigned bias_addr = (unsigned)(size_t)bias_lane;
    auto load = [&](auto qc) {
        constexpr int q = decltype(qc)::value;
        constexpr int s = SQ::slab(q);
        if constexpr (s == 0) {
            u32x4 v;
            asm volatile("ds_read_b128 %0, %1 offset:%2" : "=v"(v) : "v"(bias_addr), "n"((spec.tile0 + SQ::tile(q)) * 64));
            bias[SQ::tile(q)] = __builtin_bit_cast(f32x4, v);
        }
        if constexpr (s < NS0) a[q % PF] = __builtin_bit_cast(typename P1::frag, st.template frag<P0, G0 + q>());
        else a[q % PF] = st.template frag<P1, G0 + q>();
    };
    auto ready = [&](auto qc, auto& f) {
        constexpr int q = decltype(qc)::value;
        constexpr int F = (Q - 1 - q < PF - 1) ? Q - 1 - q : PF - 1;
        constexpr int N = F + [] { int nb = 0; for (int j = q + 1; j <= q + F; ++j) nb += SQ::slab(j) == 0; return nb; }();
        static_assert(ST::ASM_FRAGS && N >= 0 && N <= 15, "counted waits need the 16-byte asm fragment reads");
        u32x4 v = __builtin_bit_cast(u32x4, f);
        if constexpr (SQ::slab(q) == 0) asm volatile("s_waitcnt lgkmcnt(%2)" : "+v"(v), "+v"(bias[SQ::tile(q)]) : "n"(N));
        else asm volatile("s_waitcnt lgkmcnt(%1)" : "+v"(v) : "n"(N));
        f = __builtin_bit_cast(typename P1::frag, v);
    };
    static_for<0, (PF < Q ? PF : Q)>([&](auto qc) { load(qc); });
    f32x4 acc[2][2][NB];
    auto pinned = [](f32x4 v) { asm volatile("" : "+v"(v)); return v; };
    static_for<0, Q>([&](auto qc) {
        constexpr int q = decltype(qc)::value;
        constexpr int t = SQ::tile(q), s = SQ::slab(q);
        constexpr int p = t >> 1, u = t & 1, set = p & 1;
        ready(qc, a[q % PF]);
        const typename P1::frag cur = a[q % PF];
        if constexpr (q + PF < Q) load(std::integral_constant<int, q + PF>{});
        static_for<0, NB>([&](auto bc) {
            constexpr int b = decltype(bc)::value;
            const f32x4 c = (s == 0) ? bias[t] : acc[set][u][b];
            if constexpr (s < NS0) acc[set][u][b] = X16<P0>::mfma(__builtin_bit_cast(typename P0::frag, cur), in0[b][s], c);
            else acc[set][u][b] = X16<P1>::mfma(cur, in1[b][s - NS0], c);
        });
        constexpr bool host = (u == 1) || (NT % 2 == 1 && t == NT - 1);
        if constexpr (p > 0 && host && s < NB) {
            epi(std::integral_constant<int, p - 1>{}, std::integral_constant<int, s>{}, pinned(acc[set ^ 1][0][s]), pinned(acc[set ^ 1][1][s]));
        }
        if constexpr (p > 0 && host && s == NS - 1 && NS < NB) {
            static_for<NS, NB>([&](auto kc) {
                constexpr int k = decltype(kc)::value;
                epi(std::integral_constant<int, p - 1>{}, kc, pinned(acc[set ^ 1][0][k]), pinned(acc[set ^ 1][1][k]));
            });
        }
        if constexpr (q == Q - 1) {
            static_for<0, NB>([&](auto kc) {
                constexpr int k = decltype(kc)::value;
                if constexpr (u == 1) epi(std::integral_constant<int, p>{}, kc, acc[set][0][k], acc[set][1][k]);
                else epi(std::integral_constant<int, p>{}, kc, acc[set][0][k], acc[set][0][k]);
            });
        }
    });
}

template <class P, class A, int WAVES, int EPL, bool VIEWS = false, bool SAMPLE = false>
__global__ void __launch_bounds__(WAVES * 64, 1) net_kernel_x16(const NetArgs a) {
    using PL = PlanX16<P, A, VIEWS>;
    using PE = PolF16;
    using frag = typename P::frag;
    using efrag = typename PE::frag;
    constexpr int NB = X16Cfg<A>::NB, NS_H = PL::NS_H, NS_E = PL::NS_E, PFK = X16Cfg<A>::PF;
    static_assert(WAVES == X16Cfg<A>::WAVES, "launched with the architecture's own workgroup size");
    static_assert(A::L == 10, "the encoding's slot layout below is spelt out for ten frequencies (x16_enc_col)");

#ifdef NRN_TIMING
    const unsigned long long rt_kernel_start = __builtin_amdgcn_s_memrealtime();
#endif
    extern __shared__ __attribute__((aligned(16))) char smem[];
    char* ring = smem;
    float* bias_lds = (float*)(smem + RING * P::UNIT_BYTES);
    const int tid = threadIdx.x, lane = tid & 63;
    const int wave = __builtin_amdgcn_readfirstlane(tid >> 6);
    const int g = lane >> 4, n = lane & 15;
    for (int i = tid; i < PL::NTILES * 16; i += WAVES * 64) bias_lds[i] = a.bias[i];
    if (tid < 32) bias_lds[PL::NTILES * 16 + tid] = 0.0f;
    __syncthreads();
    const __attribute__((address_space(3))) f32x4* bias_lane = (const __attribute__((address_space(3))) f32x4*)(bias_lds + 4 * g);
    asm volatile("" : "+v"(bias_lane));
    WRing<P, WAVES, PL::NUP> st;
    st.init(a.wstream, ring, wave, lane);

    const int S = a.S;
    const int bpr = (S + 15) >> 4;
    const long long nblocks = (long long)a.n_rays * bpr;
    const long long per_wg = (long long)WAVES * NB;
    constexpr bool fuse = EPL > 0;
    const int RW = (bpr % NB == 0) ? 1 : ((2 * bpr) % NB == 0 ? 2 : NB);
    const int TG = RW * bpr / NB;
    const long long ngroups = ((long long)a.n_rays + WAVES * RW - 1) / (WAVES * RW);
    int* const mailbox = (int*)(bias_lds + PL::NTILES * 16 + 16);
    f32x4* const stage0 = (f32x4*)(bias_lds + PL::NTILES * 16 + 32);
    f32x4* const stage_w = stage0 + (size_t)wave * RW * bpr * 16;
    const CompositeArgs& fa = *(const CompositeArgs*)(stage0 + (size_t)WAVES * RW * bpr * 16);
    static_assert(sizeof(CompositeArgs) <= 256, "the compositing arguments' LDS slot");
    constexpr int SCR = SAMPLE ? (2 * 64 * EPL + 260) : 0;
    float* const scr_w = (float*)((char*)(stage0 + (size_t)WAVES * RW * bpr * 16) + 256) + (size_t)wave * SCR;
    if constexpr (fuse) {
        int* dst = (int*)(stage0 + (size_t)WAVES * RW * bpr * 16);
        const int* src = (const int*)&a.fuse;
        for (int i = tid; i < (int)(sizeof(CompositeArgs) / 4); i += WAVES * 64) dst[i] = src[i];
        __syncthreads();
    }
    const bool dyn = a.work_counter != nullptr;
    const int TGd = fuse ? TG : 1;
    const int tg_pub = ((-2 % TGd) + TGd) % TGd, tg_iss = ((-3 % TGd) + TGd) % TGd;
    unsigned pend = 0;
    int kseq = 0;
    long long first_id = blockIdx.x;
    if (dyn) {
        if (tid == 0) {
            mailbox[0] = (int)atomicAdd(a.work_counter, 1u);
            if (TGd == 1) { mailbox[1] = (int)atomicAdd(a.work_counter, 1u); pend = atomicAdd(a.work_counter, 1u); }
            else if (TGd == 2) pend = atomicAdd(a.work_counter, 1u);
        }
        __syncthreads();
        first_id = __builtin_amdgcn_readfirstlane(mailbox[0]);
        __syncthreads();
    }
    int tg = 0;
    long long grp = first_id;
    unsigned gdim = gridDim.x;
    asm volatile("" : "+s"(gdim));
    float cpre[NB][8];
    auto locate = [&](int tg_, long long grp_, long long b0_, int b, unsigned& so_, bool& ok_, unsigned& nb_, bool& first_) {
        bool blk_ok;
        int ray, bir;
        if constexpr (fuse) {
            const int q = tg_ * NB + b;
            const long long rr = (grp_ * WAVES + wave) * RW + q / bpr;
            blk_ok = rr < a.n_rays;
            ray = (int)(blk_ok ? rr : a.n_rays - 1);
            bir = q % bpr;
        } else {
            const long long blk_raw = b0_ + (long long)wave * NB + b;
            blk_ok = blk_raw < nblocks;
            const long long blk = blk_ok ? blk_raw : nblocks - 1;
            ray = (int)(blk / bpr);
            bir = (int)(blk % bpr);
        }
        const int sidx = bir * 16 + n;
        ok_ = blk_ok && sidx < S;
        const int sc = sidx < S ? sidx : S - 1;
        so_ = (unsigned)ray * (unsigned)S + (unsigned)sc;
        first_ = sc == 0;
        nb_ = (unsigned)ray * (unsigned)S + (unsigned)(sc == 0 ? (S > 1 ? 1 : 0) : sc - 1);
    };
    unsigned so[NB];
    bool ok[NB];
    f32x4 q4n[NB];
    f32x4 q4p[VIEWS ? NB : 1];
    bool first[NB];
    static_for<0, NB>([&](auto bc) {
        constexpr int b = decltype(bc)::value;
        unsigned nb;
        locate(0, grp, first_id * per_wg, b, so[b], ok[b], nb, first[b]);
        q4n[b] = *(const f32x4*)(a.pts4 + (size_t)so[b] * 4);
        if constexpr (VIEWS) q4p[b] = *(const f32x4*)(a.pts4 + (size_t)nb * 4);
    });
#ifdef NRN_TIMING
    unsigned long long tacc[8] = {0, 0, 0, 0, 0, 0, 0, 0};
#endif
    for (long long b0 = first_id * per_wg; fuse ? (grp < ngroups) : (b0 < nblocks); ) {
#ifdef NRN_TIMING
// ... 28 lines not shown
                ev[15] = (g == 2) ? q4[1] : 0.0f;
            }
#pragma unroll
            for (int s = 0; s < NS_E; ++s)
#pragma unroll
                for (int e = 0; e < 8; ++e) enc[b][s][e] = (_Float16)ev[8 * s + e];
        });

        efrag encv[NB][1];
        if constexpr (VIEWS) {
            static_assert(A::LV == 4, "the direction encoding's slot layout is spelt out for four frequencies (x16_dir_col)");
            static_for<0, NB>([&](auto bc) {
                constexpr int b = decltype(bc)::value;
                const f32x4 q4 = q4n[b], nb4 = q4p[b];
                float dd[3];
#pragma unroll
                for (int c = 0; c < 3; ++c) dd[c] = first[b] ? __fsub_rn(nb4[c], q4[c]) : __fsub_rn(q4[c], nb4[c]);
                const float nrm = sqrtf(__fadd_rn(__fadd_rn(__fmul_rn(dd[0], dd[0]), __fmul_rn(dd[1], dd[1])), __fmul_rn(dd[2], dd[2])));
                float dir[3], drev[3];
#pragma unroll
                for (int c = 0; c < 3; ++c) { dir[c] = __fdiv_rn(dd[c], __fadd_rn(nrm, 0.000001f)); drev[c] = dir[c] * 0.15915494309189535f; }
                float ev[8];
#pragma unroll
                for (int i = 0; i < 3; ++i) {
                    const int m = 4 * i + g;
                    const int f = m / 3, c = m - 3 * f;
                    const float xr = c == 0 ? drev[0] : (c == 1 ? drev[1] : drev[2]);
                    const float r = __builtin_amdgcn_fractf(xr * (float)(1 << f));
                    ev[2 * i] = __builtin_amdgcn_sinf(r);
                    ev[2 * i + 1] = __builtin_amdgcn_cosf(r);
                }
                ev[6] = (g == 0) ? dir[0] : (g == 1 ? dir[2] : 0.0f);
                ev[7] = (g == 0) ? dir[1] : 0.0f;
#pragma unroll
                for (int e = 0; e < 8; ++e) encv[b][0][e] = (_Float16)ev[e];
            });
        }
#ifdef NRN_TIMING
        NRN_TACC(1, t_it);
        const unsigned long long t_net = NRN_NOW();
#endif
        frag ha[NB][NS_H], hb[NB][NS_H];
        frag none[NB][1];
        auto keep = [&](auto& out) {
            return [&](auto pc, auto kc, const f32x4& d0, const f32x4& d1) {
                out[decltype(kc)::value][decltype(pc)::value] = x16_pack<P>(d0, d1);
            };
        };
        dense_x16<PE, P, PL, 0, NS_E, 0, NB, PFK>(st, bias_lane, enc, none, keep(ha));
        static_for<1, A::D>([&](auto ic) {
            constexpr int i = decltype(ic)::value;
            constexpr bool skip = (i - 1 == A::SKIP);
            if constexpr (i % 2 == 1) {
                if constexpr (skip) dense_x16<PE, P, PL, i, NS_E, NS_H, NB, PFK>(st, bias_lane, enc, ha, keep(hb));
                else dense_x16<P, P, PL, i, NS_H, 0, NB, PFK>(st, bias_lane, ha, none, keep(hb));
            } else {
                if constexpr (skip) dense_x16<PE, P, PL, i, NS_E, NS_H, NB, PFK>(st, bias_lane, enc, hb, keep(ha));
                else dense_x16<P, P, PL, i, NS_H, 0, NB, PFK>(st, bias_lane, hb, none, keep(ha));
            }
        });
        f32x4 raw[NB];
        auto take = [&](auto, auto kc, const f32x4& d0, const f32x4&) { raw[decltype(kc)::value] = d0; };
        if constexpr (!VIEWS) {
            if constexpr ((A::D - 1) % 2 == 1) dense_x16<P, P, PL, PL::L_HEAD, NS_H, 0, NB, PFK>(st, bias_lane, hb, none, take);
            else dense_x16<P, P, PL, PL::L_HEAD, NS_H, 0, NB, PFK>(st, bias_lane, ha, none, take);
        } else {
            constexpr int NS_V = PL::NS_V;
            frag hv[NB][NS_V];
            float sigma[NB];
            auto views_epi = [&](auto pc, auto kc, const f32x4& d0, const f32x4& d1) {
                constexpr int p = decltype(pc)::value, k = decltype(kc)::value;
                if constexpr (p < NS_V) hv[k][p] = x16_pack<P>(d0, d1);
                else sigma[k] = d0[0];
            };
            if constexpr ((A::D - 1) % 2 == 1) dense_x16<PE, P, PL, PL::L_VIEWS, 1, NS_H, NB, PFK>(st, bias_lane, encv, hb, views_epi);
            else dense_x16<PE, P, PL, PL::L_VIEWS, 1, NS_H, NB, PFK>(st, bias_lane, encv, ha, views_epi);
            dense_x16<P, P, PL, PL::L_HEAD, NS_V, 0, NB, PFK>(st, bias_lane, hv, none, take);
            static_for<0, NB>([&](auto bc) { raw[decltype(bc)::value][3] = sigma[decltype(bc)::value]; });
        }
#ifdef NRN_TIMING
        NRN_TACC(2, t_net);
        const unsigned long long t_out = NRN_NOW();
#endif
        static_for<PL::NUNITS, PL::NUP>([&](auto uc) { st.template advance<decltype(uc)::value>(); });
        int tg_n = tg;
        long long grp_n = grp, b0_n = b0;
        const int tgd = fuse ? tg : 0;
        long long next_id = 0;
        if (dyn) {
            if (tgd + 1 == TGd) next_id = __builtin_amdgcn_readfirstlane(mailbox[(kseq + 1) & 1]);
            if (wave == 0 && lane == 0) {
                if (tgd == tg_pub) mailbox[(kseq + (TGd == 1 ? 2 : 1)) & 1] = (int)pend;
                if (tgd == tg_iss) pend = atomicAdd(a.work_counter, 1u);
            }
            if (tgd + 1 == TGd) ++kseq;
        }
        if constexpr (fuse) {
            if (tg + 1 == TG) { tg_n = 0; grp_n = dyn ? next_id : grp + gdim; } else tg_n = tg + 1;
        } else {
            b0_n = dyn ? next_id * per_wg : b0 + (long long)gdim * per_wg;
        }
        unsigned so_n[NB];
        bool ok_n[NB];
        static_for<0, NB>([&](auto bc) {
            constexpr int b = decltype(bc)::value;
            unsigned nb;
            locate(tg_n, grp_n, b0_n, b, so_n[b], ok_n[b], nb, first[b]);
            q4n[b] = *(const f32x4*)(a.pts4 + (size_t)so_n[b] * 4);
            if constexpr (VIEWS) q4p[b] = *(const f32x4*)(a.pts4 + (size_t)nb * 4);
        });
        static_for<0, NB>([&](auto bc) {
            constexpr int b = decltype(bc)::value;
            if (ok[b] && g == 0) {
                if (!fuse) *(f32x4*)(a.raw4 + (size_t)so[b] * 4) = raw[b];
                if (a.raw_out) {
                    float* ro = a.raw_out + (size_t)so[b] * a.raw_ch;
                    ro[0] = raw[b][0]; ro[1] = raw[b][1]; ro[2] = raw[b][2]; ro[3] = raw[b][3];
                }
            }
            if (ok[b] && g == 1 && a.raw_out && a.raw_ch > 4) a.raw_out[(size_t)so[b] * a.raw_ch + 4] = raw[b][0];
            if (fuse && g == 0) stage_w[(tg * NB + b) * 16 + n] = raw[b];
        });
#ifdef NRN_TIMING
        NRN_TACC(3, t_out);
        const unsigned long long t_comp = NRN_NOW();
#endif
        if constexpr (fuse) {
            if (__builtin_expect(tg + 1 == TG, 0)) {
                static_for<0, NB>([&](auto rc) {
                    constexpr int r = decltype(rc)::value;
                    if (r < RW) {
                        const long long rr = (grp * WAVES + wave) * RW + r;
                        const bool ray_ok = rr < a.n_rays;
                        const int cray = (int)(ray_ok ? rr : a.n_rays - 1);
                        const f32x4* sw = stage_w + r * bpr * 16;
                        auto raw_at = [&](int ic) { return sw[ic]; };
                        float cz[EPL + 1], cw[EPL];
                        composite_ray<EPL, true>(fa, cray, ray_ok, lane, raw_at, cz, cw, cpre[r]);
                        if constexpr (SAMPLE) sample_merge_ray<EPL, true>(fa, cray, ray_ok, lane, cz, cw, scr_w, scr_w + 64 * EPL, scr_w + 128 * EPL);
                    }
                });
            }
        }
        tg = tg_n; grp = grp_n; b0 = b0_n;
        static_for<0, NB>([&](auto bc) { so[decltype(bc)::value] = so_n[decltype(bc)::value]; ok[decltype(bc)::value] = ok_n[decltype(bc)::value]; });
#ifdef NRN_TIMING
        NRN_TACC(4, t_comp);
        NRN_TACC(0, t_it);
        tacc[5] += __builtin_amdgcn_s_memrealtime() - r_it;
        tacc[7] += 1;
#endif
    }
    st.drain();
#ifdef NRN_TIMING
    if (blockIdx.x == 0 && lane == 0 && wave < 8) {
        tacc[6] = st.bar_cycles;
        for (int i = 0; i < 8; ++i) g_nrn_timing[wave][i] += tacc[i];
    }
    if (WAVES == 4 && lane == 0 && wave == 0 && blockIdx.x < 16) {
        const int slot = (int)blockIdx.x;
        g_nrn_timing[4 + slot / 8][slot % 8] = __builtin_amdgcn_s_memrealtime();
        if (blockIdx.x == 0) g_nrn_timing[6][0] = rt_kernel_start;
    }
#endif
}

template <class P, class A, int EPL, bool VIEWS = false, bool SAMPLE = false>
static hipError_t launch_net_x16_t(const NetArgs& a, int num_cus, hipStream_t stream) {
    constexpr int WAVES = X16Cfg<A>::WAVES;
    using PL = PlanX16<P, A, VIEWS>;
    constexpr int NB = X16Cfg<A>::NB;
    if (!a.pts4 || (!a.raw4 && !a.fuse_on) || a.S < 1) return hipErrorInvalidValue;
    if ((a.fuse_on != 0) != (EPL > 0) || (EPL > 0 && (a.S + 63) / 64 != EPL)) return hipErrorInvalidValue;
    const int bpr = (a.S + 15) / 16;
    const int RW = (bpr % NB == 0) ? 1 : ((2 * bpr) % NB == 0 ? 2 : NB);
    size_t lds = (size_t)RING * P::UNIT_BYTES + (size_t)PL::NTILES * 16 * sizeof(float) + 128;
    if (a.fuse_on) {
        if (a.S > 256 || (a.fuse.n_importance != 0) != SAMPLE || a.fuse.S != a.S) return hipErrorInvalidValue;
        lds += (size_t)WAVES * RW * bpr * 16 * 16 + 256;
        if (SAMPLE) {
            if (a.S + a.fuse.n_importance > 256 || !a.fuse.z_out) return hipErrorInvalidValue;
            lds += (size_t)WAVES * (2 * 64 * EPL + 260) * sizeof(float);
        }
    }
    if (lds > 160 * 1024) return hipErrorInvalidValue;
    auto kern = net_kernel_x16<P, A, WAVES, EPL, VIEWS, SAMPLE>;
    static bool attr_set[64] = {};
    int dev = 0;
    if (hipGetDevice(&dev) != hipSuccess) return hipErrorInvalidDevice;
    if (dev < 0 || dev >= 64 || !attr_set[dev]) {
        const size_t lds_max = (size_t)RING * P::UNIT_BYTES + (size_t)PL::NTILES * 16 * sizeof(float) + 128 + (size_t)WAVES * NB * 15 * 256 + 256 +
                               (SAMPLE ? (size_t)WAVES * (2 * 64 * EPL + 260) * sizeof(float) : 0);
        hipError_t e = hipFuncSetAttribute((const void*)kern, hipFuncAttributeMaxDynamicSharedMemorySize, (int)(lds_max < 160 * 1024 ? lds_max : 160 * 1024));
        if (e != hipSuccess) return e;
        if (dev >= 0 && dev < 64) attr_set[dev] = true;
    }
    long long want;
    if (a.fuse_on) want = ((long long)a.n_rays + WAVES * RW - 1) / (WAVES * RW);
    else want = ((long long)a.n_rays * bpr + WAVES * NB - 1) / (WAVES * NB);
    if (want <= 0) return hipSuccess;
    const int grid = (int)(want < num_cus ? want : num_cus);
    hipLaunchKernelGGL(kern, dim3(grid), dim3(WAVES * 64), lds, stream, a);
    return hipGetLastError();
}

}
```

nonrigid_nerf_amd/csrc/nrnerf_net_x16.hip:

```cpp
#include "nrnerf_net_x16.h"
#include "nrnerf_x16_api.h"

#ifndef NRN_X16_EPL
#error "compile with -DNRN_X16_EPL=0..4 (Makefile)"
#endif
#define NRN_CAT2(a, b) a##b
#define NRN_CAT(a, b) NRN_CAT2(a, b)
#ifndef NRN_X16_SAMPLE
#define NRN_X16_SAMPLE 0
#endif
#if NRN_X16_SAMPLE
#define NRN_X16_ENTRY NRN_CAT(launch_net_x16_s, NRN_X16_EPL)
#else
#define NRN_X16_ENTRY NRN_CAT(launch_net_x16_e, NRN_X16_EPL)
#endif

namespace nrn {
hipError_t NRN_X16_ENTRY(int precision, int arch, bool views, const NetArgs& a, int num_cus, hipStream_t stream) {
    constexpr bool SMP = NRN_X16_SAMPLE != 0;
    if (views) {
        if (arch != 0) return hipErrorInvalidValue;
        if (precision == PREC_BF16) return launch_net_x16_t<PolBF16, ArchDefault, NRN_X16_EPL, true, SMP>(a, num_cus, stream);
        if (precision == PREC_F16) return launch_net_x16_t<PolF16, ArchDefault, NRN_X16_EPL, true, SMP>(a, num_cus, stream);
        return hipErrorInvalidValue;
    }
    if (arch == 0) {
        if (precision == PREC_BF16) return launch_net_x16_t<PolBF16, ArchDefault, NRN_X16_EPL, false, SMP>(a, num_cus, stream);
        if (precision == PREC_F16) return launch_net_x16_t<PolF16, ArchDefault, NRN_X16_EPL, false, SMP>(a, num_cus, stream);
    } else if (arch == 5) {
        if (precision == PREC_BF16) return launch_net_x16_t<PolBF16, ArchNarrow, NRN_X16_EPL, false, SMP>(a, num_cus, stream);
        if (precision == PREC_F16) return launch_net_x16_t<PolF16, ArchNarrow, NRN_X16_EPL, false, SMP>(a, num_cus, stream);
    }
    return hipErrorInvalidValue;
}

#if NRN_X16_EPL == 0 && !NRN_X16_SAMPLE
long long x16_rays_per_group(int arch, int S) {
    const int bpr = (S + 15) / 16;
    const int NB = (arch == 5) ? X16Cfg<ArchNarrow>::NB : X16Cfg<ArchDefault>::NB, WAVES = (arch == 5) ? X16Cfg<ArchNarrow>::WAVES : X16Cfg<ArchDefault>::WAVES;
    const int RW = (bpr % NB == 0) ? 1 : ((2 * bpr) % NB == 0 ? 2 : NB);
    return (long long)WAVES * RW;
}
hipError_t launch_net_x16_e1(int, int, bool, const NetArgs&, int, hipStream_t);
hipError_t launch_net_x16_e2(int, int, bool, const NetArgs&, int, hipStream_t);
hipError_t launch_net_x16_e3(int, int, bool, const NetArgs&, int, hipStream_t);
hipError_t launch_net_x16_e4(int, int, bool, const NetArgs&, int, hipStream_t);
hipError_t launch_net_x16_s1(int, int, bool, const NetArgs&, int, hipStream_t);
hipError_t launch_net_x16_s2(int, int, bool, const NetArgs&, int, hipStream_t);
int x16_coarse_epilogue_max_samples() { return 128; }
hipError_t launch_net_x16(int precision, int arch, bool views, const NetArgs& a, int num_cus, hipStream_t stream) {
    if (!a.fuse_on) return launch_net_x16_e0(precision, arch, views, a, num_cus, stream);
    if (a.fuse.n_importance > 0) {
        switch ((a.S + 63) / 64) {
            case 1: return launch_net_x16_s1(precision, arch, views, a, num_cus, stream);
            case 2: return launch_net_x16_s2(precision, arch, views, a, num_cus, stream);
            default: return hipErrorInvalidValue;
        }
    }
    switch ((a.S + 63) / 64) {
        case 1: return launch_net_x16_e1(precision, arch, views, a, num_cus, stream);
        case 2: return launch_net_x16_e2(precision, arch, views, a, num_cus, stream);
        case 3: return launch_net_x16_e3(precision, arch, views, a, num_cus, stream);
        case 4: return launch_net_x16_e4(precision, arch, views, a, num_cus, stream);
        default: return hipErrorInvalidValue;
    }
}
#endif
}

#if defined(NRN_TIMING) && NRN_X16_EPL == 3 && !NRN_X16_SAMPLE
extern "C" int nrnerf_debug_timing_launch_net_x16(unsigned long long* out) {
    static const unsigned long long zero[64] = {};
    if (hipMemcpyFromSymbol(out, HIP_SYMBOL(nrn::g_nrn_timing), 64 * sizeof(unsigned long long)) != hipSuccess) return -1;
    return hipMemcpyToSymbol(HIP_SYMBOL(nrn::g_nrn_timing), zero, sizeof(zero)) == hipSuccess ? 0 : -1;
}
#endif
```

nonrigid_nerf_amd/csrc/nrnerf_pack.cpp:

```cpp
#include <algorithm>
#include <cstring>
#include <initializer_list>
#include <memory>
#include <stdexcept>
#include <vector>

#include "nrnerf_pack.h"
#include "nrnerf_x16_api.h"
#include "nrnerf_bend_x16_plan.h"
#include "nrnerf_plan.h"

namespace nrn {
namespace {

inline uint16_t f32_to_bf16(float f) {
    uint32_t u;
    std::memcpy(&u, &f, 4);
    if ((u & 0x7fffffffu) > 0x7f800000u) return (uint16_t)((u >> 16) | 0x40);
    u += 0x7fffu + ((u >> 16) & 1u);
    return (uint16_t)(u >> 16);
}
inline uint16_t f32_to_f16(float f) {
    _Float16 h = (_Float16)f;
    uint16_t u;
// ... 1050 lines not shown
        program(IMG_GEN_COARSE, gc, d.coarse);
        if (d.fine) program(IMG_GEN_FINE, gf, d.fine);
        if (gen_trainable(d, *d.coarse) && (!d.fine || gen_trainable(d, *d.fine))) {
            t.gen_train_ok = true;
            for (const nrnerf_mlp_desc* mlp : {d.coarse, d.fine}) {
                GenTrainNet& tn = t.gen_tn[mlp == d.coarse ? 0 : 1];
                if (!mlp) { tn = t.gen_tn[0]; continue; }
                GenProgram bw;
                gen_pack_mlp_bwd(d, *mlp, bw, lay);
                program(mlp == d.coarse ? IMG_GEN_COARSE_BWD : IMG_GEN_FINE_BWD, bw, nullptr);
                tn.W = mlp->width; tn.D = mlp->depth; tn.skip = gen_skip(*mlp) >= 0; tn.views = mlp->use_viewdirs != 0;
                tn.dv = tn.views ? 3 + 6 * d.multires_views : 0; tn.draw_col = gen_draw_col(*mlp);
                tn.in_w = mlp->time_conditioned ? mlp->pts_linears[0].in_features : 3 + 6 * d.multires; tn.lat = tn.in_w - (3 + 6 * d.multires);
            }
        }
        if (t.exact && !(t.bend_train_ok && t.gen_train_ok)) return NRNERF_ERR_UNSUPPORTED;
        if (gx16_eligible(d, *d.coarse) && (!d.fine || gx16_eligible(d, *d.fine))) {
            const bool trainable = t.gen_train_ok && gx16_trainable(d, *d.coarse) && (!d.fine || gx16_trainable(d, *d.fine));
            for (const nrnerf_mlp_desc* mlp : {d.coarse, d.fine}) {
                if (!mlp) continue;
                Image& gx = add(mlp == d.coarse ? IMG_GX_COARSE : IMG_GX_FINE);
                pack_gx16(d, *mlp, gx.pk, gx.gx, lay);
                gx.algo_flops = 2.0 * algo_macs(d2, *mlp);
                gx.mfma_flops = mfma16_flops_per_sample(gx.pk);
                gx.output_ch = mlp->output_ch;
                if (!trainable) continue;
                Image& gxb = add(mlp == d.coarse ? IMG_GX_COARSE_BWD : IMG_GX_FINE_BWD);
                pack_gx16_bwd(d, *mlp, gxb.pk, gxb.gx, lay);
            }
        }
    }
    if (t.bend_train_ok) {
        Image& fwd = add(IMG_BEND_TRAIN_FWD);
        Image& bwd = add(IMG_BEND_TRAIN_BWD);
        gen_pack_bender_train(d, cb, fwd.pk, bwd.pk, lay);
    }
    if ((t.split_ok || t.gen_compiled_bender >= 0) && bend_x16_eligible(d)) {
        Image& bx = add(IMG_BEND_X16);
        pack_bend_x16(d, bx.pk, lay);
        bx.algo_flops = bend_algo;
        bx.mfma_flops = mfma16_flops_per_sample(bx.pk);
    }
    return NRNERF_OK;
}

int pack_host_image(const nrnerf_model_desc* desc, int which, PackedPass& pk) {
    const nrnerf_mlp_desc* m = (which == 1 && desc->fine) ? desc->fine : desc->coarse;
    int rc;
    if (which == 2 || which == 3) {
        if (!desc->bender || (desc->coarse->use_viewdirs && desc->exact_viewdirs)) return NRNERF_ERR_UNSUPPORTED;
        PackedPass other;
        rc = (which == 2) ? pack_split(*desc, pk, other) : pack_split(*desc, other, pk);
    } else if (which == 4 || which == 5) {
        if (desc->coarse->time_conditioned || desc->precision == NRNERF_PREC_F16) return NRNERF_ERR_UNSUPPORTED;
        PackedPass fwd;
        nrnerf_model_desc d2 = *desc;
        d2.bender = nullptr;
        const nrnerf_mlp_desc* mm = (which == 5 && desc->fine) ? desc->fine : desc->coarse;
        int arch_id = 0;
        rc = pack_dispatch(d2, *mm, fwd, &arch_id);
        if (rc == NRNERF_OK && arch_id != 0 && arch_id != 5) rc = NRNERF_ERR_UNSUPPORTED;
        if (rc == NRNERF_OK) pack_bwd(*desc, *mm, pk);
    } else if (which == 6) {
        if (!desc->bender) return NRNERF_ERR_UNSUPPORTED;
        PackedPass fwd;
        int arch_id = 0;
        rc = pack_dispatch(*desc, *desc->coarse, fwd, &arch_id);
        if (rc == NRNERF_OK && arch_id > 1 && arch_id != 5) rc = NRNERF_ERR_UNSUPPORTED;
        if (rc == NRNERF_OK) {
            if (bender_arch(arch_id) == 0) pack_pass_bwd_bender<ArchDefault>(*desc->bender, pk);
            else pack_pass_bwd_bender<ArchDeepBend>(*desc->bender, pk);
        }
    } else if (which == 11 || which == 12) {
        const nrnerf_mlp_desc* mm = (which == 12 && desc->fine) ? desc->fine : desc->coarse;
        if (!gx16_eligible(*desc, *mm)) return NRNERF_ERR_UNSUPPORTED;
        GxMeta gm;
        rc = NRNERF_OK;
        pack_gx16(*desc, *mm, pk, gm);
    } else if (which == 10) {
        const nrnerf_mlp_desc* mm = desc->fine ? desc->fine : desc->coarse;
        if (!x16_eligible(*desc, *mm, true)) return NRNERF_ERR_UNSUPPORTED;
        rc = NRNERF_OK;
        pack_x16(*desc, *mm, pk);
    } else if (which == 13 || which == 14) {
        GenProgram gb, gc, gf;
        rc = gen_pack_all(*desc, nullptr, gb, gc, gf);
        const nrnerf_mlp_desc* mm = (which == 14) ? desc->fine : desc->coarse;
        if (rc == NRNERF_OK && !mm) rc = NRNERF_ERR_INVALID;
        if (rc == NRNERF_OK && !gen_trainable(*desc, *mm)) rc = NRNERF_ERR_UNSUPPORTED;
        if (rc == NRNERF_OK) {
            GenProgram g;
            gen_pack_mlp_bwd(*desc, *mm, g, nullptr);
            pk = g.pk;
            program_unit_table(pk, g.proto, 15, {g.proto.ke, g.proto.kv, g.proto.kh, g.proto.lat, gen_draw_col(*mm)});
        }
    } else if (which >= 7 && which <= 9) {
        GenProgram gb, gc, gf;
        rc = gen_pack_all(*desc, nullptr, gb, gc, gf);
        if (rc == NRNERF_OK && ((which == 8 && !desc->fine) || (which == 9 && !desc->bender))) rc = NRNERF_ERR_INVALID;
        if (rc == NRNERF_OK) {
            GenProgram& g = which == 7 ? gc : (which == 8 ? gf : gb);
            pk = g.pk;
            program_unit_table(pk, g.proto, 11, {g.proto.ke, g.proto.kv, g.proto.kh, g.proto.lat});
        }
    } else {
        rc = pack_dispatch(*desc, *m, pk);
    }
    return rc;
}

}
```

nonrigid_nerf_amd/csrc/nrnerf_plan.h:

```cpp
#pragma once
#include <stdint.h>

#if defined(__HIPCC__)
#define NRN_HD __host__ __device__
#else
#define NRN_HD
#endif

#ifndef NRN_UNIT_BYTES
#define NRN_UNIT_BYTES 16384
#endif
#ifndef NRN_RING
#define NRN_RING 4
#endif

namespace nrn {

constexpr NRN_HD int cdiv(int a, int b) { return (a + b - 1) / b; }
constexpr NRN_HD int imax(int a, int b) { return a > b ? a : b; }

constexpr NRN_HD int tile_row(int r, int h) { return (r & 3) + 8 * (r >> 2) + 4 * h; }

template <int KH_, bool SPLIT_ = (KH_ != 1)>
struct Shape {
    static constexpr int KH = KH_;
    static constexpr int KS = 2 * KH_;
    static constexpr int SP = 16 / KH_;
    static constexpr int ELEM_BYTES = (KH_ == 1) ? 4 : 2;
    static constexpr int FRAG_BYTES = 64 * KH_ * ELEM_BYTES;
    static constexpr bool SPLIT = SPLIT_;
    static constexpr float LO_SCALE = 2048.0f;
    static constexpr int UNIT_BYTES = NRN_UNIT_BYTES;
    static constexpr int UNIT_FRAGS = UNIT_BYTES / FRAG_BYTES;
};

template <int W_, int D_, int SKIP_, int L_, int BW_, int BD_, int RW_, int RD_, int LAT_, int LV_ = 4, int TCB_ = 0>
struct ArchT {
    static constexpr int W = W_, D = D_, SKIP = SKIP_, L = L_, LV = LV_;
    static constexpr int TCB = TCB_;
    static constexpr int BW = BW_, BD = BD_, RW = RW_, RD = RD_, LAT = LAT_;
    static_assert(W_ % 32 == 0 && BW_ % 32 == 0 && RW_ % 32 == 0, "widths must be multiples of 32");
    static_assert(LAT_ % 8 == 0, "latent size must be a multiple of 8");
};

constexpr NRN_HD int enc_F0(int L) { return (L + 1) / 2; }
constexpr NRN_HD int enc_slots(int L) { return 2 + 6 * enc_F0(L); }
constexpr NRN_HD int enc_col(int L, int h, int q) {
    if (q == 0) return h ? 2 : 0;
    if (q == 1) return h ? -1 : 1;
    int pi = (q - 2) / 2, fn = (q - 2) % 2, fl = pi / 3, c = pi % 3;
    int f = h * enc_F0(L) + fl;
    if (fl >= enc_F0(L) || f >= L) return -1;
    return 3 + 6 * f + 3 * fn + c;
}
template <class SH, class A> constexpr NRN_HD int ns_enc_xyz() { return cdiv(enc_slots(A::L), SH::KH); }
template <class SH, class A> constexpr NRN_HD int ns_trunk_in() { return ns_enc_xyz<SH, A>() + (A::TCB ? cdiv(A::LAT, 2 * SH::KH) : 0); }

constexpr NRN_HD int bin_len(int LAT) { return 8 + LAT; }
constexpr NRN_HD int bin_col(int idx, int LAT) {
    if (idx < 3) return idx;
    if (idx < 8) return -1;
    return (idx - 8 < LAT) ? 3 + (idx - 8) : -1;
}
constexpr NRN_HD int rin_len() { return 8; }
constexpr NRN_HD int rin_col(int idx) { return (idx < 3) ? idx : -1; }

enum LayerKind : int {
    LK_BEND_IN = 0, LK_BEND_HID, LK_BEND_OUT, LK_RIG_IN, LK_RIG_HID, LK_RIG_OUT,
    LK_TR_IN, LK_TR_HID, LK_TR_SKIP, LK_HEAD,
    LK_ALPHA,
    LK_FEAT,
    LK_VIEWS,
    LK_RGB,
    LK_B_HEAD,
    LK_B_HID,
    LK_B_SKIP,
    LK_B_IN,
    LK_BB_OUT,
    LK_BB_HID,
    LK_BB_IN,
    LK_BR_OUT,
    LK_BR_HID,
    LK_B_RGB,
// ... 256 lines not shown
            int q = s * KH + e;
            int c = (q < enc_slots(A::LV)) ? enc_col(A::LV, h, q) : -1;
            return c < 0 ? -1 : A::W + c;
        }
        default:         return hidden(s, 0);
    }
}
template <class SH, class A>
constexpr NRN_HD bool frag_is_f16(int kind, int s) {
    constexpr int NS_ENC = ns_trunk_in<SH, A>();
    constexpr int NS_ENCV = cdiv(enc_slots(A::LV), SH::KH);
    if (kind <= LK_RIG_OUT || kind == LK_TR_IN) return true;
    if (kind == LK_TR_SKIP) return s < NS_ENC;
    if (kind == LK_VIEWS) return s < NS_ENCV;
    return false;
}
template <class A>
constexpr NRN_HD int out_row(int kind, int t, int i, int out_features) {
    switch (kind) {
        case LK_BEND_OUT: return (i < 8 && (i & 3) < 3) ? (i & 3) : -1;
        case LK_RIG_OUT:  return (i == 0 || i == 4) ? 0 : -1;
        case LK_ALPHA:    return (i == 0 || i == 4) ? 0 : -1;
        case LK_RGB:      return (i < 8 && (i & 3) < 3) ? (i & 3) : -1;
        case LK_HEAD:     return (i < 4) ? i : ((i == 8 && out_features > 4) ? 4 : -1);
        default:          return (32 * t + i < out_features) ? 32 * t + i : -1;
    }
}

constexpr NRN_HD int x16_hidden_feature(int s, int g, int e) { return 32 * s + (e < 4 ? 4 * g + e : 16 + 4 * g + (e - 4)); }
constexpr NRN_HD int x16_enc_col_n(int L, int NSLOT, int s, int g, int e) {
    const int q = 8 * s + e, m = 4 * (q / 2) + g;
    if (m < 3 * L) return 3 + 6 * (m / 3) + 3 * (q & 1) + (m % 3);
    int spare = 0;
    for (int qq = 0; qq < q; ++qq) spare += (4 * (qq / 2) + g >= 3 * L) ? 1 : 0;
    int before = 0;
    for (int gg = 0; gg < g; ++gg)
        for (int qq = 0; qq < NSLOT; ++qq) before += (4 * (qq / 2) + gg >= 3 * L) ? 1 : 0;
    const int id = before + spare;
    return id < 3 ? id : -1;
}
constexpr NRN_HD int x16_enc_col(int L, int s, int g, int e) { return x16_enc_col_n(L, 16, s, g, e); }
constexpr NRN_HD int x16_dir_col(int LV, int g, int e) { return x16_enc_col_n(LV, 8, 0, g, e); }
template <class SH, class A, bool VIEWS = false>
constexpr Tables build_tables_x16() {
    static_assert(SH::KH == 8, "16-bit operands");
    constexpr int NT = A::W / 16, NS_H = A::W / 32, NS_E = 2;
    static_assert(3 + 6 * A::L <= 64 && A::W % 32 == 0, "the encoding fills two k-steps");
    static_assert(!VIEWS || (3 + 6 * A::LV <= 32 && A::W % 64 == 0), "the direction encoding fills one k-step");
    Tables T{};
    int nl = 0, tile0 = 0;
    auto add = [&](int kind, int index, int ns, int nt) {
        T.layers[nl] = LayerSpec{kind, index, ns, nt, tile0, 0};
        tile0 += nt;
        ++nl;
    };
    add(LK_TR_IN, 0, NS_E, NT);
    for (int i = 1; i < A::D; ++i) {
        if (i - 1 == A::SKIP) add(LK_TR_SKIP, i, NS_E + NS_H, NT);
        else add(LK_TR_HID, i, NS_H, NT);
    }
    if (VIEWS) {
        add(LK_VIEWS, 0, 1 + NS_H, NT / 2 + 1);
        add(LK_RGB, 0, NS_H / 2, 1);
    } else {
        add(LK_HEAD, 0, NS_H, 1);
    }
    T.nlayers = nl;
    T.ntiles = tile0;
    place_fragments<SH>(T);
    return T;
}
template <class SH, class A, bool VIEWS = false>
struct PlanX16 {
    static constexpr int NT = A::W / 16, NS_H = A::W / 32, NS_E = 2;
    static constexpr int NT_V = NT / 2, NS_V = NS_H / 2;
    static constexpr Tables TB = build_tables_x16<SH, A, VIEWS>();
    static constexpr int NLAYERS = TB.nlayers, NTILES = TB.ntiles, NFRAGS = TB.nfrags;
    static constexpr int NUNITS = TB.nunits, NUP = TB.nunits_padded, UF = SH::UNIT_FRAGS;
    static constexpr int MFMA_PER_BLOCK = TB.mfma_per_block;
    static_assert(TB.ntiles <= MAX_TILES && TB.nlayers <= MAX_LAYERS, "plan too large");
    static constexpr int L_HEAD = NLAYERS - 1;
    static constexpr int L_VIEWS = NLAYERS - 2;
};
template <class A>
constexpr NRN_HD int x16_out_row(int kind, int t, int r, int out_features) {
    if (kind == LK_HEAD) return r < out_features ? r : -1;
    if (kind == LK_RGB) return r < 3 ? r : -1;
    return (16 * t + r < out_features) ? 16 * t + r : -1;
}
template <class A>
constexpr NRN_HD int x16_in_col(int kind, int s, int g, int e, int in_features) {
    constexpr int IN_CH = 3 + 6 * A::L;
    if (kind == LK_TR_IN) return x16_enc_col(A::L, s, g, e);
    if (kind == LK_VIEWS) {
        constexpr int EV = 3 + 6 * A::LV;
        if (s == 0) { const int c = x16_dir_col(A::LV, g, e); return c < 0 ? -1 : (in_features - EV) + c; }
        const int c = x16_hidden_feature(s - 1, g, e);
        return c < in_features - EV ? c : -1;
    }
    if (kind == LK_TR_SKIP) {
        if (s < 2) return x16_enc_col(A::L, s, g, e);
        const int c = IN_CH + x16_hidden_feature(s - 2, g, e);
        return c < in_features ? c : -1;
    }
    const int c = x16_hidden_feature(s, g, e);
    return c < in_features ? c : -1;
}

using ArchDefault = ArchT<256, 8, 4, 10, 64, 5, 32, 3, 32>;
using ArchDeepBend = ArchT<256, 8, 4, 10, 64, 7, 32, 3, 32>;
using ArchTimeCond = ArchT<256, 8, 4, 10, 64, 5, 32, 3, 32, 4, 1>;
using ArchNarrow = ArchT<128, 8, 4, 10, 64, 5, 32, 3, 32>;
constexpr int NUM_ARCHS = 4;
template <int ID> struct ArchById { using type = ArchDefault; };
template <> struct ArchById<1> { using type = ArchDeepBend; };
template <> struct ArchById<2> { using type = ArchTimeCond; };
template <> struct ArchById<5> { using type = ArchNarrow; };
using ShapeF32 = Shape<1>;
using Shape16 = Shape<8, true>;
using Shape16Fast = Shape<8, false>;

}
```

nonrigid_nerf_amd/csrc/nrnerf_x16_api.h:

```cpp
#pragma once
#include "nrnerf_kernels.h"

namespace nrn {
hipError_t launch_net_x16(int precision, int arch, bool views, const NetArgs& a, int num_cus, hipStream_t stream);
long long x16_rays_per_group(int arch, int S);
int x16_coarse_epilogue_max_samples();
hipError_t launch_bend_x16(int arch, const BendArgs& a, int num_cus, hipStream_t stream);
struct GxArgs {
    const float* pts4;
    float* raw4;
    float* raw_out;
    int raw_ch;
    int n_rays, S;
    const void* wstream;
    const float* bias;
    int depth, skip, L;
    int n_bias_tiles;
    int LV;
    int fuse_on;
    CompositeArgs fuse;
    void* save;
    long long save_stride;
    int save_w;
    void* relu_bits;
};
constexpr int gx16_bits_bytes_per_lane(int wc) { return 4 * ((wc / 32 + 3) / 4); }
hipError_t launch_gx16(int precision, int wc, bool views, const GxArgs& a, int num_cus, hipStream_t stream);
long long gx16_rays_per_group(int wc, int S);
}
```

nonrigid_nerf_amd/render.py:

```python
from __future__ import annotations

import ctypes as C
import os
import threading
import weakref

import numpy as np
import torch

from . import _lib

_DEFAULT_PRECISION = _lib.canonical_precision(os.environ.get("NRNERF_PRECISION", "bf16"))
_SCAN_OUTPUTS = os.environ.get("NRNERF_SCAN_OUTPUTS") == "1"
_fallbacks = {}


class FallbackWarning(UserWarning):
    """A call was handed to the reference's own function saved by install() (it runs, but not on the HIP path)."""


_fallback_seen = set()


def _note_fallback(entry: str, why: str):
# ... 226 lines not shown

class Model:

    def __init__(self, network_fn, network_fine=None, precision: str | None = None, device=None, flags: int | None = None):
        self.lib = _lib.load()
        self.flags = _lib.model_flags_from_env() if flags is None else int(flags)
        self.precision = _lib.canonical_precision(precision or _DEFAULT_PRECISION)
        dev = torch.device(device if device is not None else next(network_fn.parameters()).device)
        if dev.type != "cuda":
            raise RuntimeError("nonrigid_nerf_amd renders on a ROCm device only (got %s)" % dev)
        self.device = torch.device("cuda", dev.index if dev.index is not None else torch.cuda.current_device())
        desc, keep = build_model_desc(network_fn, network_fine, self.precision, self.device.index, self.flags)
        self.has_bender = bool(desc.bender)
        self.trains_bender = bool(desc.bender) and self.precision != "f16"
        self.needs_latents = self.has_bender or bool(desc.coarse.contents.time_conditioned)
        self.latent_size = desc.bender.contents.latent_size if self.has_bender else \
            (int(getattr(network_fn, "ray_bending_latent_size", 0)) if self.needs_latents else 0)
        self.output_ch = desc.fine.contents.output_ch if desc.fine else desc.coarse.contents.output_ch
        self.coarse_output_ch = desc.coarse.contents.output_ch
        handle = C.c_void_p()
        _lib.check(self.lib.nrnerf_model_create(C.byref(desc), C.byref(handle)), "nrnerf_model_create")
        self.handle = handle
        self.generic = self.lib.nrnerf_model_is_generic(handle) == 1
        self.trains_generic = self.lib.nrnerf_model_trains_generic(handle) == 1
        if self.generic:
            self.trains_bender = self.lib.nrnerf_model_trains_bender(handle) == 1
        self._ws = {}
        self._ws_lock = threading.Lock()
        self._render_events = {}
        del keep

    def update(self, network_fn, network_fine=None) -> bool:
        desc, keep = build_model_desc(network_fn, network_fine, self.precision, self.device.index, self.flags)
        with torch.cuda.device(self.device):
            torch.cuda.synchronize(self.device)
            stream = torch.cuda.current_stream(self.device).cuda_stream
            rc = self.lib.nrnerf_model_update(self.handle, C.byref(desc), C.c_void_p(stream))
        del keep
        if rc == _lib.ERR_INVALID:
            return False
        _lib.check(rc, "nrnerf_model_update")
        return True

    def update_from_device(self, network_fn, network_fine=None) -> bool:
        with torch.cuda.device(self.device):
            cur = torch.cuda.current_stream(self.device)
            with self._ws_lock:
                pending, self._render_events = self._render_events, {}
            capturing = torch.cuda.is_current_stream_capturing()
            for sid, ev in pending.items():
                if sid != cur.cuda_stream and not capturing:
                    cur.wait_event(ev)
            ts = getattr(self, "_train_stream", None)
            if ts is not None and ts.cuda_stream != cur.cuda_stream and not capturing:
                cur.wait_stream(ts)
            flat, self._flat_state = _flat_params(network_fn, network_fine, getattr(self, "_flat_state", None))
            if flat is None or flat.device != self.device or int(self.lib.nrnerf_model_flat_size(self.handle)) != flat.numel():
                return False
            stream = cur.cuda_stream
            rc = self.lib.nrnerf_model_update_device(self.handle, C.c_void_p(flat.data_ptr()), flat.numel(), C.c_void_p(stream))
            self.note_use()
        if rc in (_lib.ERR_INVALID, _lib.ERR_UNSUPPORTED):
            return False
        _lib.check(rc, "nrnerf_model_update_device")
        return True

    def close(self):
        if getattr(self, "handle", None):
            self.lib.nrnerf_model_destroy(self.handle)
            self.handle = None

    __del__ = close

    def _workspace(self, nbytes: int, stream: int) -> torch.Tensor:
        with self._ws_lock:
            ws = self._ws.get(stream)
            if ws is None or ws.numel() < nbytes:
                ws = torch.empty(max(nbytes, 1), dtype=torch.uint8, device=self.device)
                self._ws[stream] = ws
            return ws

    def profile_begin(self):
        _lib.check(self.lib.nrnerf_profile_begin(self.handle), "nrnerf_profile_begin")

    def profile_end(self) -> dict:
        p = _lib.Profile()
        _lib.check(self.lib.nrnerf_profile_end(self.handle, C.byref(p)), "nrnerf_profile_end")
        return {name: dict(ms=p.ms[i], launches=p.launches[i], flops=p.flops[i], mfma_flops=p.mfma_flops[i], kernel=p.kernel_name[i].value.decode())
                for i, name in enumerate(_lib.KERNEL_NAMES)}

    def render(self, rays: torch.Tensor, latents: torch.Tensor | None, N_samples: int, N_importance: int = 0,
               retraw: bool = False, detailed_output: bool = False, rigidity_cutoff=None, test_time_scaling=None,
               removal_threshold=None, want_z_vals: bool = False, surface: bool = False, lindisp: bool = False,
               white_bkgd: bool = False, randoms: dict | None = None) -> dict:
        N = int(rays.shape[0])
        S, I = int(N_samples), int(N_importance)
        SF = S + I
        dev = self.device
        f32 = dict(dtype=torch.float32, device=dev)
        rays = rays.to(**f32).contiguous()
        a = _lib.RenderArgs()
        a.struct_size = C.sizeof(_lib.RenderArgs)
        a.n_rays, a.n_samples, a.n_importance = N, S, I
        a.lindisp, a.white_bkgd = int(bool(lindisp)), int(bool(white_bkgd))
        keep_alive = []
        for key, shape in (("u_coarse", (N, S)), ("noise_coarse", (N, S)), ("u_fine", (N, I)), ("noise_fine", (N, SF))):
            t = (randoms or {}).get(key)
            if t is not None:
                t = t.to(**f32).contiguous()
                if tuple(t.shape) != shape:
                    raise ValueError(f"{key} must have shape {shape}, got {tuple(t.shape)}")
                keep_alive.append(t)
                setattr(a, key, t.data_ptr())
        a.rays, a.ray_stride = rays.data_ptr(), rays.shape[1]
        if self.needs_latents:
            if latents is None:
                raise ValueError("ray_bending_latents are required (ray bender or time-conditioned baseline)")
            if latents.dim() != 2 or latents.shape[0] != N or latents.shape[1] != self.latent_size:
                raise ValueError(f"ray_bending_latents must have shape ({N}, {self.latent_size}), got {tuple(latents.shape)}")
            if latents.dim() == 2 and latents.shape[0] == N and latents.stride(0) == 0 and latents.stride(1) == 1 \
                    and latents.dtype == torch.float32 and latents.device == dev:
                a.latents, a.latent_stride = latents.data_ptr(), 0
            else:
                latents = latents.to(**f32).contiguous()
                a.latents, a.latent_stride = latents.data_ptr(), latents.shape[1]
        out = {}

        def new(key, *shape):
            t = torch.empty(*shape, **f32)
            out[key] = t
            return t.data_ptr()

        a.rgb_map, a.disp_map, a.acc_map = new("rgb_map", N, 3), new("disp_map", N), new("acc_map", N)
        if retraw:
            a.raw = new("raw", N, SF, self.output_ch if I > 0 else self.coarse_output_ch)
        if I > 0:
            a.rgb0, a.disp0, a.acc0, a.z_std = new("rgb0", N, 3), new("disp0", N), new("acc0", N), new("z_std", N)
        if want_z_vals:
            a.z_vals = new("_z_vals", N, SF)
        if surface:
            a.surface_pts, a.surface_rigidity = new("surface_pts", N, 3), new("surface_rigidity", N)
            idx = torch.empty(N, dtype=torch.int32, device=dev)
            out["median_index"] = idx
            a.median_index = idx.data_ptr()
        if detailed_output:
            def fill(so, prefix, ns):
                so.visibility_weights = new(prefix + "visibility_weights", N, ns)
                so.opacity_alpha = new(prefix + "opacity_alpha", N, ns)
                so.initial_input_pts = new(prefix + "initial_input_pts", N, ns, 3)
                so.input_pts = new(prefix + "input_pts", N, ns, 3)
                if self.has_bender:
                    so.unmasked_offsets = new(prefix + "unmasked_offsets", N, ns, 3)
                    so.masked_offsets = new(prefix + "masked_offsets", N, ns, 3)
                    so.rigidity_mask = new(prefix + "rigidity_mask", N, ns, 1)
            fill(a.coarse, "", S)
            if I > 0:
                fill(a.fine, "fine_", SF)
        a.detailed_output = int(detailed_output)
        a.flags = _lib.render_flags_from_env()
        if rigidity_cutoff is not None:
            a.has_rigidity_cutoff, a.rigidity_cutoff = 1, float(rigidity_cutoff)
        if test_time_scaling is not None:
            a.has_test_time_scaling, a.test_time_scaling = 1, float(test_time_scaling)
        if removal_threshold is not None:
            a.has_removal_threshold, a.removal_threshold = 1, float(removal_threshold)
        nbytes = self.lib.nrnerf_workspace_bytes(self.handle, N, S, I)
# ... 605 lines not shown
```

Before: 6.088 million.

## Keep input, skip and head weight fragments resident in LDS for x16 trunk

Adds a resident-slice variant of the x16 trunk kernel for the plain 256-wide, no-viewdirs, non-sampling path. The 72 fragments for the input layer, the head and the early skip slabs are loaded into LDS once per block, and only the remaining fragments stream through the weight ring. The goal is less global/L2 weight traffic and fewer ring refills per ray group. It costs extra LDS, which could lower occupancy, and the variant is used only when the total LDS fits under the cap. It also adds an opt-out flag and counters of resident launches.

```diff
diff --git a/include/nrnerf.h b/include/nrnerf.h
--- a/include/nrnerf.h
+++ b/include/nrnerf.h
@@ -136,7 +136,8 @@
     NRNERF_RENDER_BENDER_32X32 = 1u << 5,
     NRNERF_RENDER_COARSE_EPILOGUE_ON = 1u << 6,
     NRNERF_RENDER_COARSE_EPILOGUE_OFF = 1u << 7,
-    NRNERF_RENDER_FIXED_SHARES = 1u << 8
+    NRNERF_RENDER_FIXED_SHARES = 1u << 8,
+    NRNERF_RENDER_NO_RESIDENT_SLICE = 1u << 9
 } nrnerf_render_flags;
 
 #define NRNERF_NUM_KERNELS 6
@@ -426,6 +427,8 @@
 int nrnerf_composite_backward(const nrnerf_composite_args* args, void* hip_stream);
 
 int nrnerf_profile_begin(nrnerf_model* model);
+int nrnerf_resident_launches(const nrnerf_model* model, int32_t out[6]);
+size_t nrnerf_trunk_kernel_lds_bytes(int32_t precision, int32_t n_samples, int32_t fused, int32_t resident);
 int nrnerf_profile_end(nrnerf_model* model, nrnerf_profile* out);
 
 typedef enum nrnerf_visualize_flags {
diff --git a/nonrigid_nerf_amd/_lib.py b/nonrigid_nerf_amd/_lib.py
--- a/nonrigid_nerf_amd/_lib.py
+++ b/nonrigid_nerf_amd/_lib.py
@@ -77,7 +77,7 @@
 MODEL_FORCE_GENERIC, MODEL_NO_X16_F16 = 1 << 0, 1 << 1
 MODEL_PY_TRAINING_HANDLE = 1 << 30
 RENDER_FUSED_FINE_BENDER, RENDER_UNFUSED_COMPOSITE, RENDER_SPLIT_COARSE, RENDER_NO_X16, RENDER_X16_FINE_ONLY, RENDER_BENDER_32X32, \
-    RENDER_COARSE_EPILOGUE_ON, RENDER_COARSE_EPILOGUE_OFF, RENDER_FIXED_SHARES = (1 << i for i in range(9))
+    RENDER_COARSE_EPILOGUE_ON, RENDER_COARSE_EPILOGUE_OFF, RENDER_FIXED_SHARES, RENDER_NO_RESIDENT_SLICE = (1 << i for i in range(10))
 
 
 def model_flags_from_env() -> int:
@@ -90,7 +90,7 @@
 
 
 _RENDER_ENV = ("NRNERF_FUSED_FINE_BENDER", "NRNERF_UNFUSED_COMPOSITE", "NRNERF_SPLIT_COARSE", "NRNERF_X16_BENDER", "NRNERF_X16",
-               "NRNERF_FUSED_COARSE_EPILOGUE", "NRNERF_FIXED_SHARES")
+               "NRNERF_FUSED_COARSE_EPILOGUE", "NRNERF_FIXED_SHARES", "NRNERF_RESIDENT_SLICE")
 _render_flags_cache = (None, 0)
 
 
@@ -119,6 +119,8 @@
         f |= RENDER_COARSE_EPILOGUE_ON if key[5].strip() == "1" else RENDER_COARSE_EPILOGUE_OFF
     if key[6] == "1":
         f |= RENDER_FIXED_SHARES
+    if key[7] == "0":
+        f |= RENDER_NO_RESIDENT_SLICE
     _render_flags_cache = (key, f)
     return f
 
@@ -488,6 +490,8 @@
     "nrnerf_composite_forward": (C.c_int, [C.POINTER(CompositeArgs), C.c_void_p]),
     "nrnerf_composite_backward": (C.c_int, [C.POINTER(CompositeArgs), C.c_void_p]),
     "nrnerf_profile_begin": (C.c_int, [C.c_void_p]),
+    "nrnerf_resident_launches": (C.c_int, [C.c_void_p, C.POINTER(C.c_int32)]),
+    "nrnerf_trunk_kernel_lds_bytes": (C.c_size_t, [C.c_int32, C.c_int32, C.c_int32, C.c_int32]),
     "nrnerf_profile_end": (C.c_int, [C.c_void_p, C.POINTER(Profile)]),
     "nrnerf_visualize_frames": (C.c_int, [C.POINTER(VisualizeArgs), C.c_void_p]),
     "nrnerf_visualize_workspace_bytes": (C.c_size_t, [C.c_int32, C.c_int32, C.c_int32]),
diff --git a/nonrigid_nerf_amd/csrc/nrnerf_api.cpp b/nonrigid_nerf_amd/csrc/nrnerf_api.cpp
--- a/nonrigid_nerf_amd/csrc/nrnerf_api.cpp
+++ b/nonrigid_nerf_amd/csrc/nrnerf_api.cpp
@@ -450,6 +450,11 @@
             return timed(ev, [&] {
                 if (p.net != NetFamily::NetX16) return launch_net(m->precision, p.net == NetFamily::NetBender, m->views, p.dispatch, n, m->num_cus, stream);
                 n.work_counter = counter(p.trunk_counter, (size_t)16 * BEND_COUNTERS_PER_LAUNCH * 2 + 16 * p.which);
+                n.no_resident = (a->flags & NRNERF_RENDER_NO_RESIDENT_SLICE) ? 1 : 0;
+                if (x16_takes_resident(m->precision, p.dispatch, m->views, n)) {
+                    std::lock_guard<std::mutex> g(m->prof_mu);
+                    ++m->resident_launches[p.net_slot];
+                }
                 return launch_net_x16(m->precision, p.dispatch, m->views, n, m->num_cus, stream);
             });
         }
@@ -745,9 +750,23 @@
     std::lock_guard<std::mutex> g(m->prof_mu);
     for (auto& e : m->prof_events) { (void)hipEventDestroy(e.a); (void)hipEventDestroy(e.b); }
     m->prof_events.clear();
+    for (int& n : m->resident_launches) n = 0;
     m->prof_on = true;
     return NRNERF_OK;
 } NRN_CATCH
+
+int nrnerf_resident_launches(const nrnerf_model* m, int32_t out[6]) try {
+    if (!m || !out) return NRNERF_ERR_INVALID;
+    std::lock_guard<std::mutex> g(m->prof_mu);
+    for (int i = 0; i < NRNERF_NUM_KERNELS; ++i) out[i] = m->resident_launches[i];
+    return NRNERF_OK;
+} NRN_CATCH
+
+size_t nrnerf_trunk_kernel_lds_bytes(int32_t precision, int32_t n_samples, int32_t fused, int32_t resident) {
+    const int prec = precision == NRNERF_PREC_BF16 ? PREC_BF16 : (precision == NRNERF_PREC_F16 ? PREC_F16 : -1);
+    if (prec < 0 || n_samples < 1 || n_samples > NRNERF_MAX_SAMPLES) return 0;
+    return x16_lds_request(prec, 0, false, n_samples, fused != 0, false, resident != 0);
+}
 
 int nrnerf_profile_end(nrnerf_model* m, nrnerf_profile* out) try {
     if (!m || !out) return NRNERF_ERR_INVALID;
diff --git a/nonrigid_nerf_amd/csrc/nrnerf_kernels.h b/nonrigid_nerf_amd/csrc/nrnerf_kernels.h
--- a/nonrigid_nerf_amd/csrc/nrnerf_kernels.h
+++ b/nonrigid_nerf_amd/csrc/nrnerf_kernels.h
@@ -87,6 +87,7 @@
     int fuse_on;
     CompositeArgs fuse;
     unsigned* work_counter;
+    int no_resident;
 };
 
 
diff --git a/nonrigid_nerf_amd/csrc/nrnerf_model.h b/nonrigid_nerf_amd/csrc/nrnerf_model.h
--- a/nonrigid_nerf_amd/csrc/nrnerf_model.h
+++ b/nonrigid_nerf_amd/csrc/nrnerf_model.h
@@ -53,6 +53,7 @@
     unsigned* adam_barrier = nullptr;
     mutable std::mutex prof_mu;
     mutable bool prof_on = false;
+    mutable int resident_launches[NRNERF_NUM_KERNELS] = {};
     struct Ev { int kernel; hipEvent_t a, b; double flops, mfma; const char* name; };
     mutable std::vector<Ev> prof_events;
 };
diff --git a/nonrigid_nerf_amd/csrc/nrnerf_net_impl.h b/nonrigid_nerf_amd/csrc/nrnerf_net_impl.h
--- a/nonrigid_nerf_amd/csrc/nrnerf_net_impl.h
+++ b/nonrigid_nerf_amd/csrc/nrnerf_net_impl.h
@@ -108,7 +108,7 @@
     else asm volatile("s_waitcnt vmcnt(%0)" ::"n"(N) : "memory");
 }
 
-template <class P, int WAVES, int NUP>
+template <class P, int WAVES, int NUP, class SRC = void>
 struct WRing {
     static constexpr int UNIT = P::UNIT_BYTES;
     static constexpr int PW = UNIT / 1024 / WAVES;
@@ -137,7 +137,9 @@
     }
     template <int V>
     __device__ __forceinline__ void issue() {
-        unsigned off = (unsigned)(V * UNIT);
+        unsigned off;
+        if constexpr (std::is_void<SRC>::value) off = (unsigned)(V * UNIT);
+        else off = (unsigned)SRC::unit_src_bytes(V);
         asm volatile("" : "+s"(off));
         const char* src = (ubase + off) + lane16;
         char* dst = ring + (V % RING) * UNIT + wave_off;
@@ -162,6 +164,10 @@
     static constexpr bool ASM_FRAGS = (P::FRAG_BYTES == 1024);
     template <class PX, int GF>
     __device__ __forceinline__ typename PX::frag frag() {
+        return ring_frag<PX, GF>();
+    }
+    template <class PX, int GF>
+    __device__ __forceinline__ typename PX::frag ring_frag() {
         static_assert(PX::FRAG_BYTES == P::FRAG_BYTES, "mixed policies must share the fragment size");
         constexpr int UF = P::UNIT_FRAGS;
         if constexpr (GF % UF == 0) advance<GF / UF>();
@@ -186,6 +192,50 @@
         }
     }
     __device__ __forceinline__ void drain() { asm volatile("s_waitcnt vmcnt(0)" ::: "memory"); }
+};
+
+template <class P, int WAVES, class RS>
+struct WRingRes : WRing<P, WAVES, RS::NUNITS, RS> {
+    using Base = WRing<P, WAVES, RS::NUNITS, RS>;
+    static constexpr bool RESIDENT = true;
+    static constexpr int SPAN = 65536 / P::FRAG_BYTES;
+    static constexpr int NBASE = (RS::NRES + SPAN - 1) / SPAN;
+    static_assert(Base::ASM_FRAGS && RS::NRES % WAVES == 0, "16-byte asm fragment reads; the block splits evenly over the waves");
+    unsigned res_addr[NBASE];
+
+    template <int G> static constexpr bool is_resident() { return RS::resident(G); }
+    __device__ __forceinline__ void init(const void* stream, char* lds, char* block, int wave, int lane) {
+        Base::init(stream, lds, wave, lane);
+        const char* const src0 = (const char*)stream + wave * P::FRAG_BYTES + this->lane16;
+        char* const dst0 = block + wave * P::FRAG_BYTES;
+        static_for<0, RS::NRES / WAVES>([&](auto cc) {
+            constexpr int c = decltype(cc)::value;
+            static_assert(RS::T.res_src[c * WAVES + WAVES - 1] == RS::T.res_src[c * WAVES] + WAVES - 1, "a run of WAVES resident slots is contiguous in the image");
+            unsigned off = (unsigned)(RS::T.res_src[c * WAVES] * P::FRAG_BYTES);
+            asm volatile("" : "+s"(off));
+            __builtin_amdgcn_global_load_lds((const __attribute__((address_space(1))) void*)(src0 + off),
+                                             (__attribute__((address_space(3))) void*)(dst0 + c * WAVES * P::FRAG_BYTES), 16, 0, 0);
+        });
+        static_for<0, NBASE>([&](auto ic) {
+            constexpr int i = decltype(ic)::value;
+            res_addr[i] = (unsigned)(size_t)(__attribute__((address_space(3))) char*)block + (unsigned)this->lane_off + (unsigned)(i * SPAN * P::FRAG_BYTES);
+            asm volatile("" : "+v"(res_addr[i]));
+        });
+        asm volatile("s_waitcnt vmcnt(0)" ::: "memory");
+        __syncthreads();
+    }
+    template <class PX, int GF>
+    __device__ __forceinline__ typename PX::frag frag() {
+        if constexpr (RS::resident(GF)) {
+            static_assert(PX::FRAG_BYTES == P::FRAG_BYTES, "mixed policies must share the fragment size");
+            constexpr int R = RS::T.res_of[GF];
+            u32x4 v;
+            asm volatile("ds_read_b128 %0, %1 offset:%2" : "=v"(v) : "v"(res_addr[R / SPAN]), "n"((R % SPAN) * P::FRAG_BYTES));
+            return __builtin_bit_cast(typename PX::frag, v);
+        } else {
+            return Base::template ring_frag<PX, RS::T.ring_of[GF]>();
+        }
+    }
 };
 
 typedef const __attribute__((address_space(3))) f32x4* BiasPtr;
diff --git a/nonrigid_nerf_amd/csrc/nrnerf_net_x16.h b/nonrigid_nerf_amd/csrc/nrnerf_net_x16.h
--- a/nonrigid_nerf_amd/csrc/nrnerf_net_x16.h
+++ b/nonrigid_nerf_amd/csrc/nrnerf_net_x16.h
@@ -25,6 +25,9 @@
     }
     return __builtin_bit_cast(typename P::frag, w);
 }
+
+template <class ST, class = void> struct x16_has_resident : std::false_type {};
+template <class ST> struct x16_has_resident<ST, typename std::enable_if<ST::RESIDENT>::type> : std::true_type {};
 
 #ifndef NRN_X16_NB
 #define NRN_X16_NB 4
@@ -68,6 +71,8 @@
             asm volatile("ds_read_b128 %0, %1 offset:%2" : "=v"(v) : "v"(bias_addr), "n"((spec.tile0 + SQ::tile(q)) * 64));
             bias[SQ::tile(q)] = __builtin_bit_cast(f32x4, v);
         }
+        if constexpr (x16_has_resident<ST>::value) static_assert(ST::template is_resident<G0 + q>() == (spec.kind == LK_TR_IN || spec.kind == LK_HEAD || (spec.kind == LK_TR_SKIP && s < NS0)),
+                                                  "resident-slice table and SeqPos disagree");
         if constexpr (s < NS0) a[q % PF] = __builtin_bit_cast(typename P1::frag, st.template frag<P0, G0 + q>());
         else a[q % PF] = st.template frag<P1, G0 + q>();
     };
@@ -117,9 +122,12 @@
     });
 }
 
-template <class P, class A, int WAVES, int EPL, bool VIEWS = false, bool SAMPLE = false>
+template <class A, bool VIEWS, bool SAMPLE> struct X16Res { static constexpr bool OK = !VIEWS && !SAMPLE && A::W == 256; };
+template <class P, class A, int WAVES, int EPL, bool VIEWS = false, bool SAMPLE = false, bool RES = false>
 __global__ void __launch_bounds__(WAVES * 64, 1) net_kernel_x16(const NetArgs a) {
     using PL = PlanX16<P, A, VIEWS>;
+    using RS = ResX16<P, A>;
+    static_assert(!RES || X16Res<A, VIEWS, SAMPLE>::OK, "the resident slice: plain head, no coarse epilogue, the 256-wide trunk");
     using PE = PolF16;
     using frag = typename P::frag;
     using efrag = typename PE::frag;
@@ -132,7 +140,12 @@
 #endif
     extern __shared__ __attribute__((aligned(16))) char smem[];
     char* ring = smem;
-    float* bias_lds = (float*)(smem + RING * P::UNIT_BYTES);
+    size_t res_bytes = 0;
+    if constexpr (RES) {
+        static_assert(RS::NRES == 72 && RS::NRING == 896 && RS::NUNITS == 56 && RS::NUNITS % RING == 0, "7 x 128 ring fragments = 56 units; 32 + 32 + 8 resident");
+        res_bytes = RS::BYTES;
+    }
+    float* bias_lds = (float*)(smem + RING * P::UNIT_BYTES + res_bytes);
     const int tid = threadIdx.x, lane = tid & 63;
     const int wave = __builtin_amdgcn_readfirstlane(tid >> 6);
     const int g = lane >> 4, n = lane & 15;
@@ -141,8 +154,9 @@
     __syncthreads();
     const __attribute__((address_space(3))) f32x4* bias_lane = (const __attribute__((address_space(3))) f32x4*)(bias_lds + 4 * g);
     asm volatile("" : "+v"(bias_lane));
-    WRing<P, WAVES, PL::NUP> st;
-    st.init(a.wstream, ring, wave, lane);
+    typename std::conditional<RES, WRingRes<P, WAVES, RS>, WRing<P, WAVES, PL::NUP>>::type st;
+    if constexpr (RES) st.init(a.wstream, ring, smem + RING * P::UNIT_BYTES, wave, lane);
+    else st.init(a.wstream, ring, wave, lane);
 
     const int S = a.S;
     const int bpr = (S + 15) >> 4;
@@ -337,7 +351,7 @@
         NRN_TACC(2, t_net);
         const unsigned long long t_out = NRN_NOW();
 #endif
-        static_for<PL::NUNITS, PL::NUP>([&](auto uc) { st.template advance<decltype(uc)::value>(); });
+        if constexpr (!RES) static_for<PL::NUNITS, PL::NUP>([&](auto uc) { st.template advance<decltype(uc)::value>(); });
         int tg_n = tg;
         long long grp_n = grp, b0_n = b0;
         const int tgd = fuse ? tg : 0;
@@ -420,6 +434,35 @@
 #endif
 }
 
+template <class P, class A, bool VIEWS>
+static size_t x16_launch_lds(int S, bool fused, bool sample, bool resident) {
+    size_t res_bytes = 0;
+    if constexpr (X16Res<A, VIEWS, false>::OK) res_bytes = resident ? (size_t)ResX16<P, A>::BYTES : 0;
+    return x16_lds_bytes(P::UNIT_BYTES, PlanX16<P, A, VIEWS>::NTILES, X16Cfg<A>::WAVES, X16Cfg<A>::NB, S, fused, sample, res_bytes);
+}
+template <class P, class A, bool VIEWS, bool SAMPLE>
+static bool x16_resident_fits(const NetArgs& a) {
+    if (!X16Res<A, VIEWS, SAMPLE>::OK || a.no_resident) return false;
+    return x16_launch_lds<P, A, VIEWS>(a.S, a.fuse_on != 0, SAMPLE, true) <= X16_LDS_MAX;
+}
+template <class P, class A, int EPL, bool VIEWS, bool SAMPLE, bool RES>
+static hipError_t x16_launch_kernel(const NetArgs& a, size_t lds, int grid, hipStream_t stream) {
+    constexpr int WAVES = X16Cfg<A>::WAVES, NB = X16Cfg<A>::NB;
+    auto kern = net_kernel_x16<P, A, WAVES, EPL, VIEWS, SAMPLE, RES>;
+    static bool attr_set[64] = {};
+    int dev = 0;
+    if (hipGetDevice(&dev) != hipSuccess) return hipErrorInvalidDevice;
+    if (dev < 0 || dev >= 64 || !attr_set[dev]) {
+        const size_t lds_max = x16_launch_lds<P, A, VIEWS>(0, false, false, RES) + (size_t)WAVES * NB * 15 * 256 + 256 +
+                               (SAMPLE ? (size_t)WAVES * (2 * 64 * EPL + 260) * sizeof(float) : 0);
+        hipError_t e = hipFuncSetAttribute((const void*)kern, hipFuncAttributeMaxDynamicSharedMemorySize, (int)(lds_max < X16_LDS_MAX ? lds_max : X16_LDS_MAX));
+        if (e != hipSuccess) return e;
+        if (dev >= 0 && dev < 64) attr_set[dev] = true;
+    }
+    hipLaunchKernelGGL(kern, dim3(grid), dim3(WAVES * 64), lds, stream, a);
+    return hipGetLastError();
+}
+
 template <class P, class A, int EPL, bool VIEWS = false, bool SAMPLE = false>
 static hipError_t launch_net_x16_t(const NetArgs& a, int num_cus, hipStream_t stream) {
     constexpr int WAVES = X16Cfg<A>::WAVES;
@@ -429,34 +472,21 @@
     if ((a.fuse_on != 0) != (EPL > 0) || (EPL > 0 && (a.S + 63) / 64 != EPL)) return hipErrorInvalidValue;
     const int bpr = (a.S + 15) / 16;
     const int RW = (bpr % NB == 0) ? 1 : ((2 * bpr) % NB == 0 ? 2 : NB);
-    size_t lds = (size_t)RING * P::UNIT_BYTES + (size_t)PL::NTILES * 16 * sizeof(float) + 128;
     if (a.fuse_on) {
         if (a.S > 256 || (a.fuse.n_importance != 0) != SAMPLE || a.fuse.S != a.S) return hipErrorInvalidValue;
-        lds += (size_t)WAVES * RW * bpr * 16 * 16 + 256;
-        if (SAMPLE) {
-            if (a.S + a.fuse.n_importance > 256 || !a.fuse.z_out) return hipErrorInvalidValue;
-            lds += (size_t)WAVES * (2 * 64 * EPL + 260) * sizeof(float);
-        }
-    }
-    if (lds > 160 * 1024) return hipErrorInvalidValue;
-    auto kern = net_kernel_x16<P, A, WAVES, EPL, VIEWS, SAMPLE>;
-    static bool attr_set[64] = {};
-    int dev = 0;
-    if (hipGetDevice(&dev) != hipSuccess) return hipErrorInvalidDevice;
-    if (dev < 0 || dev >= 64 || !attr_set[dev]) {
-        const size_t lds_max = (size_t)RING * P::UNIT_BYTES + (size_t)PL::NTILES * 16 * sizeof(float) + 128 + (size_t)WAVES * NB * 15 * 256 + 256 +
-                               (SAMPLE ? (size_t)WAVES * (2 * 64 * EPL + 260) * sizeof(float) : 0);
-        hipError_t e = hipFuncSetAttribute((const void*)kern, hipFuncAttributeMaxDynamicSharedMemorySize, (int)(lds_max < 160 * 1024 ? lds_max : 160 * 1024));
-        if (e != hipSuccess) return e;
-        if (dev >= 0 && dev < 64) attr_set[dev] = true;
-    }
+        if (SAMPLE && (a.S + a.fuse.n_importance > 256 || !a.fuse.z_out)) return hipErrorInvalidValue;
+    }
+    const size_t lds = x16_launch_lds<P, A, VIEWS>(a.S, a.fuse_on != 0, SAMPLE, false);
+    if (lds > X16_LDS_MAX) return hipErrorInvalidValue;
     long long want;
     if (a.fuse_on) want = ((long long)a.n_rays + WAVES * RW - 1) / (WAVES * RW);
     else want = ((long long)a.n_rays * bpr + WAVES * NB - 1) / (WAVES * NB);
     if (want <= 0) return hipSuccess;
     const int grid = (int)(want < num_cus ? want : num_cus);
-    hipLaunchKernelGGL(kern, dim3(grid), dim3(WAVES * 64), lds, stream, a);
-    return hipGetLastError();
-}
-
-}
+    if constexpr (X16Res<A, VIEWS, SAMPLE>::OK) {
+        if (x16_resident_fits<P, A, VIEWS, SAMPLE>(a)) return x16_launch_kernel<P, A, EPL, VIEWS, SAMPLE, true>(a, x16_launch_lds<P, A, VIEWS>(a.S, a.fuse_on != 0, SAMPLE, true), grid, stream);
+    }
+    return x16_launch_kernel<P, A, EPL, VIEWS, SAMPLE, false>(a, lds, grid, stream);
+}
+
+}
diff --git a/nonrigid_nerf_amd/csrc/nrnerf_net_x16.hip b/nonrigid_nerf_amd/csrc/nrnerf_net_x16.hip
--- a/nonrigid_nerf_amd/csrc/nrnerf_net_x16.hip
+++ b/nonrigid_nerf_amd/csrc/nrnerf_net_x16.hip
@@ -41,6 +41,20 @@
     const int RW = (bpr % NB == 0) ? 1 : ((2 * bpr) % NB == 0 ? 2 : NB);
     return (long long)WAVES * RW;
 }
+bool x16_takes_resident(int precision, int arch, bool views, const NetArgs& a) {
+    if (views || arch != 0 || (a.fuse_on && a.fuse.n_importance > 0)) return false;
+    if (precision == PREC_BF16) return x16_resident_fits<PolBF16, ArchDefault, false, false>(a);
+    if (precision == PREC_F16) return x16_resident_fits<PolF16, ArchDefault, false, false>(a);
+    return false;
+}
+size_t x16_lds_request(int precision, int arch, bool views, int S, bool fused, bool sample, bool resident) {
+    if ((precision != PREC_BF16 && precision != PREC_F16) || (arch != 0 && arch != 5) || (views && arch != 0) || S < 1) return 0;
+    if (resident && (views || sample || arch != 0)) return 0;
+    if (arch == 5) return x16_launch_lds<PolBF16, ArchNarrow, false>(S, fused, sample, false);
+    if (views) return x16_launch_lds<PolBF16, ArchDefault, true>(S, fused, sample, false);
+    if (precision == PREC_BF16) return x16_launch_lds<PolBF16, ArchDefault, false>(S, fused, sample, resident);
+    return x16_launch_lds<PolF16, ArchDefault, false>(S, fused, sample, resident);
+}
 hipError_t launch_net_x16_e1(int, int, bool, const NetArgs&, int, hipStream_t);
 hipError_t launch_net_x16_e2(int, int, bool, const NetArgs&, int, hipStream_t);
 hipError_t launch_net_x16_e3(int, int, bool, const NetArgs&, int, hipStream_t);
diff --git a/nonrigid_nerf_amd/csrc/nrnerf_pack.cpp b/nonrigid_nerf_amd/csrc/nrnerf_pack.cpp
--- a/nonrigid_nerf_amd/csrc/nrnerf_pack.cpp
+++ b/nonrigid_nerf_amd/csrc/nrnerf_pack.cpp
@@ -1156,6 +1156,23 @@
         if (!x16_eligible(*desc, *mm, true)) return NRNERF_ERR_UNSUPPORTED;
         rc = NRNERF_OK;
         pack_x16(*desc, *mm, pk);
+    } else if (which == 15) {
+        const nrnerf_mlp_desc* mm = desc->fine ? desc->fine : desc->coarse;
+        if (!x16_eligible(*desc, *mm, true) || mm->use_viewdirs || mm->width != 256) return NRNERF_ERR_UNSUPPORTED;
+        rc = NRNERF_OK;
+        auto table = [&](auto rs) {
+            using RS = decltype(rs);
+            pk = PackedPass{};
+            pk.frag_bytes = Shape16::FRAG_BYTES; pk.slot_bytes = Shape16::UNIT_BYTES;
+            pk.unit_off.assign(1, (uint32_t)RS::NRES);
+            for (int r = 0; r < RS::NRES; ++r) pk.unit_off.push_back((uint32_t)RS::T.res_src[r]);
+            pk.unit_off.push_back((uint32_t)RS::NUNITS);
+            pk.unit_off.push_back((uint32_t)Shape16::UNIT_FRAGS);
+            for (int u = 0; u < RS::NUNITS; ++u) pk.unit_off.push_back((uint32_t)(RS::unit_src_bytes(u) / 16));
+            pk.nunits = (int)pk.unit_off.size() - 1;
+        };
+        if (desc->precision == NRNERF_PREC_F16) table(ResX16<Shape16, ArchDefault>{});
+        else table(ResX16<Shape16Fast, ArchDefault>{});
     } else if (which == 13 || which == 14) {
         GenProgram gb, gc, gf;
         rc = gen_pack_all(*desc, nullptr, gb, gc, gf);
diff --git a/nonrigid_nerf_amd/csrc/nrnerf_plan.h b/nonrigid_nerf_amd/csrc/nrnerf_plan.h
--- a/nonrigid_nerf_amd/csrc/nrnerf_plan.h
+++ b/nonrigid_nerf_amd/csrc/nrnerf_plan.h
@@ -1,4 +1,5 @@
 #pragma once
+#include <stddef.h>
 #include <stdint.h>
 
 #if defined(__HIPCC__)
@@ -421,6 +422,65 @@
     static constexpr int L_HEAD = NLAYERS - 1;
     static constexpr int L_VIEWS = NLAYERS - 2;
 };
+struct ResTable {
+    static constexpr int MAXF = 1024, MAXU = 64, MAXR = 96;
+    short res_of[MAXF];
+    short ring_of[MAXF];
+    short res_src[MAXR];
+    short unit_src[MAXU];
+    int nres, nring, nunits;
+    bool whole_units;
+};
+template <class SH, class A>
+constexpr ResTable build_res_table() {
+    using PL = PlanX16<SH, A, false>;
+    static_assert(PL::NFRAGS <= ResTable::MAXF, "table sizes");
+    ResTable R{};
+    bool whole = true;
+    int g = 0;
+    for (int l = 0; l < PL::TB.nlayers; ++l) {
+        const LayerSpec spec = PL::TB.layers[l];
+        const int npair = spec.nt / 2, Q = spec.nt * spec.ns;
+        for (int q = 0; q < Q; ++q, ++g) {
+            const int slab = q < npair * 2 * spec.ns ? (q % (2 * spec.ns)) / 2 : q - npair * 2 * spec.ns;
+            const bool res = spec.kind == LK_TR_IN || spec.kind == LK_HEAD || (spec.kind == LK_TR_SKIP && slab < PL::NS_E);
+            R.res_of[g] = -1; R.ring_of[g] = -1;
+            if (res) {
+                if (R.nres < ResTable::MAXR) R.res_src[R.nres] = (short)g;
+                R.res_of[g] = (short)R.nres++;
+            } else {
+                const int u = R.nring / SH::UNIT_FRAGS, k = R.nring % SH::UNIT_FRAGS;
+                if (k == 0 && u < ResTable::MAXU) R.unit_src[u] = (short)g;
+                if (u >= ResTable::MAXU || g != R.unit_src[u] + k) whole = false;
+                R.ring_of[g] = (short)R.nring++;
+            }
+        }
+    }
+    R.nunits = R.nring / SH::UNIT_FRAGS;
+    R.whole_units = whole && R.nring % SH::UNIT_FRAGS == 0 && R.nres <= ResTable::MAXR && g == PL::NFRAGS;
+    return R;
+}
+template <class SH, class A>
+struct ResX16 {
+    static constexpr ResTable T = build_res_table<SH, A>();
+    static constexpr int NRES = T.nres, NRING = T.nring, NUNITS = T.nunits;
+    static constexpr int BYTES = NRES * SH::FRAG_BYTES;
+    static_assert(T.whole_units, "every ring unit is one contiguous UNIT_BYTES run of the image");
+    static_assert(NRES + NRING == PlanX16<SH, A, false>::NFRAGS, "resident and ring fragments partition the image");
+    static_assert(NUNITS % RING == 0 && NUNITS >= RING, "the ring carries whole periods: unit 0 lands in slot 0 without padding units");
+    static constexpr bool resident(int g) { return T.res_of[g] >= 0; }
+    static constexpr int unit_src_bytes(int v) { return T.unit_src[v] * SH::FRAG_BYTES; }
+};
+constexpr NRN_HD size_t x16_lds_bytes(int unit_bytes, int ntiles, int waves, int nb, int S, bool fused, bool sample, size_t resident_bytes) {
+    const int bpr = (S + 15) / 16, epl = (S + 63) / 64;
+    const int rw = (bpr % nb == 0) ? 1 : ((2 * bpr) % nb == 0 ? 2 : nb);
+    size_t lds = (size_t)RING * unit_bytes + resident_bytes + (size_t)ntiles * 16 * sizeof(float) + 128;
+    if (fused) lds += (size_t)waves * rw * bpr * 16 * 16 + 256;
+    if (fused && sample) lds += (size_t)waves * (2 * 64 * epl + 260) * sizeof(float);
+    return lds;
+}
+constexpr size_t X16_LDS_MAX = 160 * 1024;
+
 template <class A>
 constexpr NRN_HD int x16_out_row(int kind, int t, int r, int out_features) {
     if (kind == LK_HEAD) return r < out_features ? r : -1;
diff --git a/nonrigid_nerf_amd/csrc/nrnerf_x16_api.h b/nonrigid_nerf_amd/csrc/nrnerf_x16_api.h
--- a/nonrigid_nerf_amd/csrc/nrnerf_x16_api.h
+++ b/nonrigid_nerf_amd/csrc/nrnerf_x16_api.h
@@ -3,6 +3,8 @@
 
 namespace nrn {
 hipError_t launch_net_x16(int precision, int arch, bool views, const NetArgs& a, int num_cus, hipStream_t stream);
+bool x16_takes_resident(int precision, int arch, bool views, const NetArgs& a);
+size_t x16_lds_request(int precision, int arch, bool views, int S, bool fused, bool sample, bool resident);
 long long x16_rays_per_group(int arch, int S);
 int x16_coarse_epilogue_max_samples();
 hipError_t launch_bend_x16(int arch, const BendArgs& a, int num_cus, hipStream_t stream);
diff --git a/nonrigid_nerf_amd/render.py b/nonrigid_nerf_amd/render.py
--- a/nonrigid_nerf_amd/render.py
+++ b/nonrigid_nerf_amd/render.py
@@ -332,6 +332,11 @@
 
     def profile_begin(self):
         _lib.check(self.lib.nrnerf_profile_begin(self.handle), "nrnerf_profile_begin")
+
+    def resident_launches(self) -> dict:
+        n = (C.c_int32 * len(_lib.KERNEL_NAMES))()
+        _lib.check(self.lib.nrnerf_resident_launches(self.handle, n), "nrnerf_resident_launches")
+        return {name: int(n[i]) for i, name in enumerate(_lib.KERNEL_NAMES)}
 
     def profile_end(self) -> dict:
         p = _lib.Profile()
```

After: 6.156 million, median of 6. +1.1%, better.
